# AgentMaker/PAPC

Measured on AMD Instinct MI355X. Metric: point-clouds/sec (fwd+bwd) PointNet++SSG B=32 N=4096, higher is better.
Workload: dtype f32

## Files before the change

include/papc_hip.h:

```cpp
#ifndef PAPC_HIP_H
#define PAPC_HIP_H

#include <stddef.h>
#include <stdint.h>

#ifdef __cplusplus
extern "C" {
#endif

#define PAPC_OK 0
#define PAPC_E_INVALID (-1)
#define PAPC_E_UNSUPPORTED (-2)
#define PAPC_E_LAUNCH (-3)

typedef void *papc_stream_t;

int papc_version(void);
#define PAPC_ABI_VERSION 8
int papc_abi_version(void);
int64_t papc_abi_sizeof(const char *struct_name);
const char *papc_last_error_string(void);


int papc_fps_f32(const float *xyz, int64_t sb, int64_t sn, int64_t sc, int B, int N, int npoint,
// ... 108 lines not shown
int papc_bn_eval_consts_f32(const float *running_mean, const float *running_var, const float *gamma, const float *beta,
                            float eps, int C, float *mean, float *invstd, float *scale, float *shift,
                            papc_stream_t stream);

int papc_group_max_bwd_f32(const float *gout, const int32_t *argmax, int64_t G, int K, int C, float *dx,
                           papc_stream_t stream);

typedef struct papc_bwd_dy {
    int dz_mode;
    const float *dz;
    const float *gout;
    const int32_t *argmax;
    int K;
    const float *y;
    const float *mean, *invstd, *scale, *shift, *c1, *c2;
    const float *wrow;
    const int32_t *seg_grp;
    const int32_t *rows_dev;
    const float *psel;
} papc_bwd_dy;

typedef struct papc_scatter_dst {
    float *grad_feats;
    const int32_t *idx;
    int N, S, K, D;
    int col0;
} papc_scatter_dst;
typedef struct papc_bwd_red {
    const float *y;
    const float *mean, *invstd, *scale, *shift;
    float *red_partial;
    int32_t store_masked;
} papc_bwd_red;
int papc_mlp_bwd_dx_f32(const papc_bwd_dy *dy, const float *wt, int64_t M, int Cin, int Cout, float *dx,
                        const papc_scatter_dst *scatter, const papc_bwd_red *next_red, papc_stream_t stream);

int papc_mlp_bwd_dw_f32(const papc_bwd_dy *dy, int a_mode, const float *x, int64_t ldx,
                        const papc_group_src *grp, const float *bn_scale, const float *bn_shift, int64_t M,
                        int Cin, int Cout, int rows_per_chunk, float *dw_partial, float *db_partial,
                        int64_t part_ld, papc_stream_t stream);

int papc_mlp_bwd_dw_chunk_hint(int64_t M, int Cin, int Cout, int a_mode, int dz_mode, int K);

int papc_reduce_partials_f32(const float *partial, int n_chunks, int64_t n, float *out, int accumulate,
                             papc_stream_t stream);
typedef struct papc_reduce_job {
    const float *partial;
    int32_t n_chunks;
    int32_t accumulate;
    int64_t ld, n1, n2;
    float *out1, *out2;
} papc_reduce_job;
int papc_reduce_partials_batch_f32(const papc_reduce_job *jobs, int count, papc_stream_t stream);
int papc_reduce_partials2_f32(const float *partial, int n_chunks, int64_t ld, int64_t n1, float *out1, int64_t n2,
                              float *out2, int accumulate, papc_stream_t stream);

#define PAPC_FOLD_MAX 24
typedef struct papc_fold_job {
    const float *partial;
    int32_t n_chunks;
    int32_t accumulate;
    int64_t ld;
    int32_t rows, cols;
    float *out; int64_t out_ld;
} papc_fold_job;
typedef struct papc_fold_list { papc_fold_job *jobs; int32_t capacity, count; } papc_fold_list;
int papc_fold_jobs_f32(const papc_fold_job *jobs, int count, papc_stream_t stream);

#define PAPC_SA_MAX_LAYERS 8
#define PAPC_SA_IN_GROUP 0
#define PAPC_SA_IN_ROWS 1
#define PAPC_SA_NO_LINGATHER 1u
#define PAPC_SA_NO_XYZ1 2u
#define PAPC_SA_NO_NOSTORE 4u
#define PAPC_SA_NO_GMAX 8u
#define PAPC_SA_NO_FUSED_RED 16u
#define PAPC_SA_NO_COMPACT 32u
#define PAPC_SA_NO_PLANES 64u
#define PAPC_SA_NO_PLANES_POINTWISE 128u
#define PAPC_SA_NO_XYZ_FUSE 256u
#define PAPC_SA_NO_PSEL 1024u
#define PAPC_SA_NO_GSIGN 2048u
#define PAPC_SA_NO_WSTATS 512u
typedef struct papc_sa_desc {
    int32_t B, N, S, K, D;
    int32_t n_layers;
    int32_t cin;
    int32_t cout[PAPC_SA_MAX_LAYERS];
    int32_t input;
    int32_t identity_rows;
    int32_t xyz_first, pool, eval_bn, cut_gather_grad;
    float eps, momentum;
    uint32_t disable;
    int32_t inference;
    int32_t want_input_grad;
} papc_sa_desc;
typedef struct papc_sa_layer {
    const float *w, *b, *gamma, *beta;
    float *running_mean, *running_var;
} papc_sa_layer;
typedef struct papc_compact_src {
    const int32_t *start, *rows, *cidx, *seg_grp;
    const float *wrow, *coef;
    int32_t G;
} papc_compact_src;
typedef struct papc_sa_io {
    const float *xyz; int64_t sb, sn, sc;
    const float *new_xyz;
    const float *feats;
    const int32_t *idx;
    const float *x_rows;
    const float *xc; const double *xc_gram;
    const papc_compact_src *compact;
    const float *consts3; int32_t consts3_ld;
    papc_sa_layer layer[PAPC_SA_MAX_LAYERS];
    float *out;
    void *saved, *scratch;
    const papc_point_lists *plists;
    const float *wfeat;
} papc_sa_io;
typedef struct papc_sa_plan {
    papc_sa_desc d;
    int32_t cin0;
    int32_t lin0, xyz1, gmax, nostore, compact, sparse_max, planes;
    int64_t saved_bytes, fwd_scratch_bytes, bwd_scratch_bytes;
    int64_t off_y[PAPC_SA_MAX_LAYERS], off_cst[PAPC_SA_MAX_LAYERS], off_argmax;
} papc_sa_plan;
typedef struct papc_sa_grads {
    const float *gout;
    float *dw[PAPC_SA_MAX_LAYERS], *db[PAPC_SA_MAX_LAYERS], *dgamma[PAPC_SA_MAX_LAYERS], *dbeta[PAPC_SA_MAX_LAYERS];
    int32_t acc_w[PAPC_SA_MAX_LAYERS], acc_gb[PAPC_SA_MAX_LAYERS];
    const float *wt[PAPC_SA_MAX_LAYERS];
    float *grad_feats, *grad_x;
    struct papc_fold_list *defer;
} papc_sa_grads;
int papc_sa_mlp_plan(const papc_sa_desc *desc, const papc_sa_io *io, papc_sa_plan *plan);
int papc_sa_mlp_fwd(const papc_sa_plan *plan, const papc_sa_io *io, papc_stream_t stream);
int papc_sa_mlp_bwd(const papc_sa_plan *plan, const papc_sa_io *io, const papc_sa_grads *grads, papc_stream_t stream);

typedef struct papc_pfn_desc {
    int32_t P, T, C;
    float vx, vy, x_offset, y_offset;
    float eps, momentum;
    int32_t training;
    int32_t zero_padded;
} papc_pfn_desc;
typedef struct papc_pfn_io {
    const float *features; const int32_t *num_voxels, *coors;
    const float *w, *gamma, *beta;
    float *running_mean, *running_var;
    float *out;
    void *saved, *scratch;
    uint32_t *tickets;
} papc_pfn_io;
int papc_pfn_workspace(const papc_pfn_desc *desc, int64_t *saved_bytes, int64_t *scratch_bytes);
int papc_pfn_fwd(const papc_pfn_desc *desc, const papc_pfn_io *io, papc_stream_t stream);
int papc_pfn_bwd(const papc_pfn_desc *desc, const papc_pfn_io *io, const float *gout, float *dw, float *dgamma, float *dbeta, int accumulate,
                 papc_stream_t stream);


int papc_pfn_decorate_f32(const float *features, const int32_t *num_voxels, const int32_t *coors, int P, int T,
                          float vx, float vy, float x_offset, float y_offset, int with_distance, float *out,
                          papc_stream_t stream);
int papc_pfn_decorate_nf_f32(const float *features, int F, const int32_t *num_voxels, const int32_t *coors, int P, int T,
                             float vx, float vy, float x_offset, float y_offset, int with_distance, float *out, papc_stream_t stream);
int papc_pfn_stats_f32(const float *features, const int32_t *num_voxels, const int32_t *coors, int P, int T,
// ... 22 lines not shown
                               float *running_mean, float *running_var, double *gram, papc_stream_t stream);
int papc_pfn_bwd_sparse_f32(const float *features, const int32_t *num_voxels, const int32_t *coors, int P,
                            int T, float vx, float vy, float x_offset, float y_offset, const float *w, int C,
                            const float *gout, const int32_t *argmax, const float *mean, const float *invstd,
                            const float *scale, const float *shift, float *partial, papc_stream_t stream);
int papc_pfn_bwd_finalize_f32(const float *sums, int64_t M, const float *w, int C, const double *gram, const float *mean,
                              const float *invstd, const float *scale, float *dgamma, float *dbeta, float *dw, int flags,
                              papc_stream_t stream);


size_t papc_points_to_voxel_workspace(int N);
int papc_points_to_voxel_f32(const float *points, int N, int ndim, const float *voxel_size, const float *coors_range,
                             int max_points, int max_voxels, int reverse_index, float *voxels, int32_t *coors,
                             int32_t *num_points, int32_t *voxel_num, void *workspace, size_t workspace_bytes,
                             papc_stream_t stream);

int papc_pillar_scatter_f32(const float *voxel_features, const int32_t *coords, int P, int C, int batch_size, int ny,
                            int nx, float *canvas, int32_t *owner, papc_stream_t stream);
int papc_pillar_scatter_bwd_f32(const float *grad_canvas, const int32_t *coords, const int32_t *owner, int P, int C,
                                int batch_size, int ny, int nx, float *grad_features, papc_stream_t stream);

int papc_head_fc_f32(const float *x, const float *w, const float *bias, const float *gamma, const float *beta, int B, int Cin, int Cout,
                     int has_bn, float eps, float momentum, float *running_mean, float *running_var, int64_t *num_batches_tracked,
                     float drop_p, const int64_t *rng_state, int layer_tag, int64_t *rng_bump, float *y, float *mean, float *invstd,
                     uint8_t *keep, float *out, papc_stream_t stream);
int papc_head_bwd_f32(const float *gnext, const float *wnext, int Cn, const float *out, const float *y, const float *mean,
                      const float *invstd, const float *gamma, float drop_p, int has_bn, const float *x, int B, int Cin, int Cout,
                      float *dy, float *dw, float *db, float *dgamma, float *dbeta, int accumulate, papc_stream_t stream);
int papc_softmax_xent_f32(const float *logits, const int64_t *labels, int B, int C, float *loss, float *dlogits, papc_stream_t stream);

typedef struct papc_head_fc_layer {
    const float *x, *w, *bias, *gamma, *beta;
    int32_t Cin, Cout, has_bn;
    float eps, momentum;
    float *running_mean, *running_var; int64_t *num_batches_tracked;
    float drop_p; int32_t layer_tag;
    float *y, *mean, *invstd; uint8_t *keep; float *out;
} papc_head_fc_layer;
typedef struct papc_head_bwd_job {
    const float *gnext, *wnext; int32_t Cn;
    const float *out, *y, *mean, *invstd, *gamma; float drop_p; int32_t has_bn;
    const float *x; int32_t Cin, Cout;
    float *dy, *dw, *db, *dgamma, *dbeta; int32_t accumulate;
    int32_t phase;
} papc_head_bwd_job;
int papc_head_chain_fwd_f32(const papc_head_fc_layer *layers, int n_layers, int B, const int64_t *rng_state, int64_t *rng_bump,
                            const int64_t *labels, float *loss, float *dlogits, uint32_t *sync, papc_stream_t stream);
int papc_head_chain_bwd_f32(const papc_head_bwd_job *jobs, int n_jobs, int B, uint32_t *sync, papc_stream_t stream);

int papc_cloud_transform_f32(const float *x, int64_t sb, int64_t sn, int64_t sc, const float *T, int64_t ldt, int B, int N, int C, float *y,
                             papc_stream_t stream);
size_t papc_cloud_transform_bwd_workspace(int B, int N, int C);
int papc_cloud_transform_bwd_f32(const float *x, int64_t sb, int64_t sn, int64_t sc, const float *T, int64_t ldt, const float *dy, int B, int N, int C,
                                 float *dx, int64_t dsb, int64_t dsn, int64_t dsc, int accumulate, float *dT, void *workspace,
                                 size_t workspace_bytes, papc_stream_t stream);

int papc_cloud_concat_conv_parts(int B, int N);
int papc_cloud_concat_conv_f32(const float *x, int64_t ldx, const float *g, const float *w, const float *bias, int B, int N, int Cp, int Cg, int Cout,
                               float *y, float *cvec, float *stats_partial, papc_stream_t stream);
size_t papc_cloud_concat_conv_bwd_workspace(int B, int N, int Cp, int Cg, int Cout);
int papc_cloud_concat_conv_bwd_f32(const float *dz, const float *y, const float *mean, const float *invstd, const float *scale, const float *shift,
                                   const float *c1, const float *c2, const float *x, int64_t ldx, const float *g, const float *w, int B, int N, int Cp,
                                   int Cg, int Cout, float *dx, int64_t ldd, int accumulate, float *dw, float *dbias, float *dg, float *s_out,
                                   void *workspace, size_t workspace_bytes, papc_stream_t stream);

size_t papc_nms_workspace(int N);
int papc_nms_f32(const float *dets, int N, float nms_overlap_thresh, int32_t *keep, int32_t *num_out, void *workspace,
                 size_t workspace_bytes, papc_stream_t stream);
int papc_rotate_nms_f32(const float *dets, int N, float nms_overlap_thresh, int32_t *keep, int32_t *num_out, void *workspace,
                        size_t workspace_bytes, papc_stream_t stream);
int papc_rotate_iou_f32(const float *boxes, const float *query_boxes, int N, int K, int criterion, float *iou, papc_stream_t stream);
int papc_rbbox_iou_f32(const float *box_corners, const float *qbox_corners, const float *standup_iou, float standup_thresh, int N, int K,
                       float *overlaps, papc_stream_t stream);
int papc_riou_f32(const float *rbboxes, const float *qrbboxes, float standup_thresh, int N, int K, float *overlaps, papc_stream_t stream);

int papc_lingather_parts(int64_t M);
int papc_mlp_compact_ok(int64_t M, int K, int n_layers, const int *couts);
int papc_compact_plan_f32(const int32_t *idx, int G, int K, int32_t *cnt8, int32_t *start, int32_t *rows, int32_t *cidx, int32_t *seg_grp,
                          float *wrow, float *coef, papc_stream_t stream);
int papc_compact_corr_parts(void);
int papc_bn_stats_corr_f32(const float *y, int C, const int32_t *start, const float *coef, int G, float *stats_rows, papc_stream_t stream);
int papc_bn_relu_max_seg_f32(const float *y, int C, const int32_t *start, const float *scale, const float *shift, int G, float *out,
                             int32_t *argmax, float *ysel, papc_stream_t stream);
int papc_lingather_fwd_f32(const float *P, const papc_group_src *grp, int B, const float *w, int ldw, int xcol0, const float *bias, int C,
                           float *y, float *stats_partial, papc_stream_t stream);
int papc_lingather_bwd_f32(const papc_bwd_dy *dy, const papc_group_src *grp, int B, int C, float *G, float *dwx_partial, papc_stream_t stream);
int papc_lingather_bwd_pp_ok(const papc_group_src *grp, int B, int C);
int papc_lingather_bwd_pp_f32(const papc_bwd_dy *dy, const papc_group_src *grp, int B, int C, const float *P, const float *w, int ldw, int xcol0,
                              const float *bias, float *G, float *dwx_partial, papc_stream_t stream);
int papc_lingather_list_parts(int64_t BN);
int papc_lingather_bwd_parts(const papc_group_src *grp, int B, int C);
int papc_lingather_bwd_lists_ok(const papc_group_src *grp, int C);
int papc_point_lists_f32(const papc_group_src *grp, int B, const int32_t *start, int32_t *prange, int32_t *prow, float *pmeta, float *pmom,
                         papc_stream_t stream);

int papc_mlp_bwd_dx_xyz_ok(int64_t M, int Cin, int Cout);
int papc_mlp_bwd_dx_xyz_f32(const papc_bwd_dy *dy, const float *wt, int64_t M, int Cin, int Cout, const float *xc, const float *wf,
                            float *partial, papc_stream_t stream);

int papc_bn_max_prep_f32(const float *gout, const float *ysel, const float *scale, const float *shift, const float *mean,
                         const float *invstd, const float *c1, const float *c2, const float *w, const float *bias, int64_t G, int Co,
                         int Ci, float *psel, float *wcat, float *hbias, float *e_out, float *q_out, papc_stream_t stream);
int papc_mlp_bwd_dx_max_f32(const float *psel, const int32_t *argmax, int K, const float *x, int64_t ldx, const float *bn_scale,
                            const float *bn_shift, const float *wcat, const float *hbias, int64_t M, int Cin, int Cout, float *dx,
                            const papc_bwd_red *next_red, papc_stream_t stream);

int papc_mlp_max_nostore_ok(int64_t M, int Cin, int Cout, int K);
int64_t papc_mlp_bwd_dw_max_ws_floats(int64_t M, int Cin, int Cout);
int papc_mlp_bwd_dw_max_f32(const float *psel, const int32_t *argmax, int K, const float *x, const float *bn_scale, const float *bn_shift,
                            const float *w, const float *e, const float *scale, const float *c1, int64_t M, int Cin, int Cout,
                            float *workspace, float *dw, int accumulate, papc_stream_t stream);

int papc_mlp_xyz_ok(int64_t M, int C1, int C2);
int papc_xyz_parts(int64_t M);
int papc_xyz_bwd_parts(int64_t M);
int papc_xyz_group_f32(const papc_group_src *grp, int B, float *xc, double *gram_partial, papc_stream_t stream);
int papc_xyz_gram_fold_f32(const double *gram_partial, int parts, double *gram, papc_stream_t stream);
int papc_xyz_l1_finalize_f32(const double *gram_partial, int parts, int64_t M, const float *w, int ldw, int xcol0, const float *bias,
                             const float *gamma, const float *beta, float eps, float momentum, int C, float *mean, float *invstd, float *scale,
                             float *shift, float *running_mean, float *running_var, float *wf, double *gram, papc_stream_t stream);
int papc_xyz_l1_bwd_f32(const float *dz, const float *xc, const float *wf, int64_t M, int C, float *partial, papc_stream_t stream);
int papc_xyz_l1_bwd_finalize_f32(const float *partial, int parts, int64_t M, int C, const double *gram, const float *w, int ldw, int xcol0,
                                 const float *bias, const float *mean, const float *invstd, const float *scale, float *dgamma, float *dbeta,
                                 float *dw, int accumulate, papc_stream_t stream);

size_t papc_pg_planes_bytes(int64_t R, int64_t K);

typedef struct papc_pg_wjob {
    const float *src;
    int64_t row_stride, col_stride;
    int R, K;
    void *planes;
} papc_pg_wjob;
int papc_pg_prep_weights_f32(const papc_pg_wjob *jobs, int count, papc_stream_t stream);

#define PAPC_PG_PLAIN 0
#define PAPC_PG_CONCAT 1
#define PAPC_PG_BNRELU 2
#define PAPC_PG_DY_DENSE 3
#define PAPC_PG_DY_MAX 4
typedef struct papc_pg_prep {
    int mode;
    int64_t M; int C;
    const float *x; int64_t ldx;
    const float *xyz; int64_t sb, sn, sc; const float *feats; int N, D, xyz_first;
    const float *dz;
    const float *gout, *ysel; const int32_t *argmax; int K;
    const float *stats; int parts;
    const float *gamma, *beta; float eps, momentum; float *running_mean, *running_var;
    float *mean, *invstd, *scale, *shift;
    const float *red; int red_parts;
    float *dgamma, *dbeta; int accumulate;
    void *planes, *planes_t;
} papc_pg_prep;
int papc_pg_prep_rows_f32(const papc_pg_prep *args, papc_stream_t stream);

#define PAPC_PG_STORE 0
#define PAPC_PG_FWD 1
#define PAPC_PG_FWD_GMAX 2
#define PAPC_PG_RED 3
typedef struct papc_pg_gemm {
    int epi;
    const void *a, *b;
    int R1, R2, K;
    float *c; int64_t ldc;
    int split; int64_t split_stride;
// ... 77 lines not shown
```

papc_amd/_lib.py:

```python
import ctypes
import os

_HERE = os.path.dirname(os.path.abspath(__file__))
LIB_PATH = os.environ.get("PAPC_LIB") or os.path.join(_HERE, "libpapc_hip.so")

ABI_VERSION = 8

c_p = ctypes.c_void_p
c_i = ctypes.c_int
c_l = ctypes.c_int64
c_f = ctypes.c_float


class PapcError(RuntimeError):
    pass


class GroupSrc(ctypes.Structure):
    _fields_ = [("xyz", c_p), ("sb", c_l), ("sn", c_l), ("sc", c_l), ("new_xyz", c_p), ("feats", c_p),
                ("idx", c_p), ("N", c_i), ("S", c_i), ("K", c_i), ("D", c_i), ("xyz_first", c_i),
                ("cidx", c_p), ("seg_grp", c_p), ("rows_dev", c_p), ("wstat", c_p), ("plists", c_p)]


class PointLists(ctypes.Structure):
    _fields_ = [("prange", c_p), ("prow", c_p), ("pmeta", c_p), ("compact", c_i), ("pmom", c_p)]


class BwdDy(ctypes.Structure):
    _fields_ = [("dz_mode", c_i), ("dz", c_p), ("gout", c_p), ("argmax", c_p), ("K", c_i), ("y", c_p),
                ("mean", c_p), ("invstd", c_p), ("scale", c_p), ("shift", c_p), ("c1", c_p), ("c2", c_p),
                ("wrow", c_p), ("seg_grp", c_p), ("rows_dev", c_p), ("psel", c_p)]


class GroupMax(ctypes.Structure):
    _fields_ = [("gmax", c_p), ("gmin", c_p), ("amax", c_p), ("amin", c_p), ("K", c_i), ("sign_src", c_p)]


class BwdRed(ctypes.Structure):
    _fields_ = [("y", c_p), ("mean", c_p), ("invstd", c_p), ("scale", c_p), ("shift", c_p), ("red_partial", c_p), ("store_masked", c_i)]


class CopyJob(ctypes.Structure):
    _fields_ = [("src", ctypes.c_void_p), ("dst", ctypes.c_void_p), ("B", ctypes.c_int32), ("R", ctypes.c_int32), ("C", ctypes.c_int32),
                ("sb", ctypes.c_int64), ("sr", ctypes.c_int64), ("sc", ctypes.c_int64), ("db", ctypes.c_int64), ("dr", ctypes.c_int64),
                ("dc", ctypes.c_int64)]


class ReduceJob(ctypes.Structure):
    _fields_ = [("partial", c_p), ("n_chunks", ctypes.c_int32), ("accumulate", ctypes.c_int32), ("ld", c_l), ("n1", c_l), ("n2", c_l),
                ("out1", c_p), ("out2", c_p)]


class ScatterDst(ctypes.Structure):
    _fields_ = [("grad_feats", c_p), ("idx", c_p), ("N", c_i), ("S", c_i), ("K", c_i), ("D", c_i), ("col0", c_i)]


SIGNATURES = {
    "papc_version": (c_i, []),
    "papc_abi_version": (c_i, []),
    "papc_abi_sizeof": (c_l, [ctypes.c_char_p]),
    "papc_last_error_string": (ctypes.c_char_p, []),
    "papc_fps_f32": (c_i, [c_p, c_l, c_l, c_l, c_i, c_i, c_i, c_p, c_f, c_p, c_p, c_p]),
    "papc_ball_query_f32": (c_i, [c_p, c_l, c_l, c_l, c_p, c_i, c_i, c_i, c_i, c_p, c_p, c_p, c_i, c_p]),
    "papc_square_distance_f32": (c_i, [c_p, c_p, c_i, c_i, c_i, c_p, c_p]),
    "papc_index_points_f32": (c_i, [c_p, c_p, c_i, c_i, c_i, c_i, c_i, c_p, c_p]),
    "papc_index_points_bwd_f32": (c_i, [c_p, c_p, c_i, c_i, c_i, c_i, c_i, c_p, c_p]),
    "papc_group_points_f32": (c_i, [c_p, c_l, c_l, c_l, c_p, c_p, c_p, c_i, c_i, c_i, c_i, c_i, c_i, c_p, c_p]),
    "papc_group_points_bwd_f32": (c_i, [c_p, c_p, c_i, c_i, c_i, c_i, c_i, c_i, c_p, c_p, c_p, c_p]),
    "papc_three_nn_f32": (c_i, [c_p, c_l, c_l, c_l, c_p, c_l, c_l, c_l, c_i, c_i, c_i, c_p, c_p, c_p, c_p]),
    "papc_three_interpolate_f32": (c_i, [c_p, c_p, c_p, c_i, c_i, c_i, c_i, c_p, c_p]),
    "papc_three_interpolate_bwd_f32": (c_i, [c_p, c_p, c_p, c_i, c_i, c_i, c_i, c_p, c_p]),
    "papc_three_interpolate_bwd_first3_f32": (c_i, [c_p, c_p, c_i, c_i, c_i, c_i, c_p, c_p]),
    "papc_mlp_gemm_parts": (c_i, [c_l]),
    "papc_mlp_gemm_gmax_ok": (c_i, [c_l, c_i, c_i]),
    "papc_mlp_gemm_f32": (c_i, [c_i, c_p, c_l, c_p, c_p, c_p, c_p, c_p, c_l, c_i, c_i, c_p, c_p, c_p, c_p]),
    "papc_mlp_gemm_rows_f32": (c_i, [c_i, c_p, c_l, c_p, c_p, c_p, c_p, c_p, c_l, c_i, c_i, c_p, c_p, c_p, c_p, c_p]),
    "papc_mlp_gemm_rows_w_f32": (c_i, [c_i, c_p, c_l, c_p, c_p, c_p, c_p, c_p, c_l, c_i, c_i, c_p, c_p, c_p, c_p, c_p, c_p]),
    "papc_sa_mlp_plan": (c_i, [c_p, c_p, c_p]),
    "papc_sa_mlp_fwd": (c_i, [c_p, c_p, c_p]),
    "papc_sa_mlp_bwd": (c_i, [c_p, c_p, c_p, c_p]),
    "papc_pfn_workspace": (c_i, [c_p, c_p, c_p]),
    "papc_pfn_fwd": (c_i, [c_p, c_p, c_p]),
    "papc_pfn_bwd": (c_i, [c_p, c_p, c_p, c_p, c_p, c_p, c_i, c_p]),
    "papc_compact_plan_f32": (c_i, [c_p, c_i, c_i, c_p, c_p, c_p, c_p, c_p, c_p, c_p, c_p]),
    "papc_compact_corr_parts": (c_i, []),
    "papc_mlp_compact_ok": (c_i, [c_l, c_i, c_i, c_p]),
    "papc_bn_stats_corr_f32": (c_i, [c_p, c_i, c_p, c_p, c_i, c_p, c_p]),
    "papc_bn_relu_max_seg_f32": (c_i, [c_p, c_i, c_p, c_p, c_p, c_i, c_p, c_p, c_p, c_p]),
    "papc_bn_select_max_f32": (c_i, [c_p, c_p, c_p, c_p, c_p, c_p, c_l, c_i, c_p, c_p, c_p]),
    "papc_bn_finalize_f32": (c_i, [c_p, c_i, c_l, c_i, c_p, c_p, c_f, c_f, c_p, c_p, c_p, c_p, c_p, c_p, c_p]),
    "papc_bn_relu_max_f32": (c_i, [c_p, c_p, c_p, c_l, c_i, c_i, c_p, c_p, c_p]),
    "papc_bn_relu_f32": (c_i, [c_p, c_p, c_p, c_l, c_i, c_p, c_p]),
    "papc_bn_bwd_reduce_max_f32": (c_i, [c_p, c_p, c_i, c_p, c_p, c_p, c_p, c_l, c_i, c_i, c_p, c_p, c_p]),
    "papc_bn_bwd_reduce_f32": (c_i, [c_i, c_p, c_p, c_p, c_i, c_p, c_p, c_p, c_p, c_p, c_l, c_i, c_i, c_p, c_p]),
    "papc_bn_bwd_finalize_f32": (c_i, [c_p, c_i, c_l, c_i, c_p, c_p, c_p, c_p, c_i, c_p]),
    "papc_bn_eval_consts_f32": (c_i, [c_p, c_p, c_p, c_p, c_f, c_i, c_p, c_p, c_p, c_p, c_p]),
    "papc_group_max_bwd_f32": (c_i, [c_p, c_p, c_l, c_i, c_i, c_p, c_p]),
    "papc_mlp_bwd_dx_f32": (c_i, [c_p, c_p, c_l, c_i, c_i, c_p, c_p, c_p, c_p]),
    "papc_mlp_bwd_dw_f32": (c_i, [c_p, c_i, c_p, c_l, c_p, c_p, c_p, c_l, c_i, c_i, c_i, c_p, c_p, c_l, c_p]),
    "papc_reduce_partials2_f32": (c_i, [c_p, c_i, c_l, c_l, c_p, c_l, c_p, c_i, c_p]),
    "papc_reduce_partials_batch_f32": (c_i, [c_p, c_i, c_p]),
    "papc_fold_jobs_f32": (c_i, [c_p, c_i, c_p]),
    "papc_mlp_bwd_dw_chunk_hint": (c_i, [c_l, c_i, c_i, c_i, c_i, c_i]),
    "papc_reduce_partials_f32": (c_i, [c_p, c_i, c_l, c_p, c_i, c_p]),
    "papc_pfn_decorate_f32": (c_i, [c_p, c_p, c_p, c_i, c_i, c_f, c_f, c_f, c_f, c_i, c_p, c_p]),
    "papc_pfn_decorate_nf_f32": (c_i, [c_p, c_i, c_p, c_p, c_i, c_i, c_f, c_f, c_f, c_f, c_i, c_p, c_p]),
    "papc_pfn_stats_f32": (c_i, [c_p, c_p, c_p, c_i, c_i, c_f, c_f, c_f, c_f, c_p, c_i, c_p, c_p, c_p]),
    "papc_pfn_apply_f32": (c_i, [c_p, c_p, c_p, c_i, c_i, c_f, c_f, c_f, c_f, c_p, c_i, c_p, c_p, c_p, c_p, c_p]),
    "papc_pfn_num_blocks": (c_i, [c_i]),
    "papc_pfn_bwd_reduce_f32": (c_i, [c_p, c_p, c_p, c_i, c_i, c_f, c_f, c_f, c_f, c_p, c_i, c_p, c_p, c_p, c_p, c_p, c_p, c_p, c_p]),
    "papc_pfn_bwd_dw_f32": (c_i, [c_p, c_p, c_p, c_i, c_i, c_f, c_f, c_f, c_f, c_p, c_i, c_p, c_p, c_p, c_p, c_p, c_p, c_p, c_p, c_p, c_p]),
    "papc_pfn_gram_blocks": (c_i, [c_i]),
    "papc_pfn_gram_f32": (c_i, [c_p, c_p, c_p, c_i, c_i, c_f, c_f, c_f, c_f, c_p, c_p]),
    "papc_pfn_gram_finalize_f32": (c_i, [c_p, c_i, c_l, c_p, c_i, c_p, c_p, c_f, c_f, c_p, c_p, c_p, c_p, c_p, c_p, c_p, c_p]),
    "papc_pfn_bwd_sparse_f32": (c_i, [c_p, c_p, c_p, c_i, c_i, c_f, c_f, c_f, c_f, c_p, c_i, c_p, c_p, c_p, c_p, c_p, c_p, c_p, c_p]),
    "papc_pfn_bwd_finalize_f32": (c_i, [c_p, c_l, c_p, c_i, c_p, c_p, c_p, c_p, c_p, c_p, c_p, c_i, c_p]),
    "papc_points_to_voxel_workspace": (ctypes.c_size_t, [c_i]),
    "papc_points_to_voxel_f32": (c_i, [c_p, c_i, c_i, c_p, c_p, c_i, c_i, c_i, c_p, c_p, c_p, c_p, c_p, ctypes.c_size_t, c_p]),
    "papc_pillar_scatter_f32": (c_i, [c_p, c_p, c_i, c_i, c_i, c_i, c_i, c_p, c_p, c_p]),
    "papc_pillar_scatter_bwd_f32": (c_i, [c_p, c_p, c_p, c_i, c_i, c_i, c_i, c_i, c_p, c_p]),
    "papc_head_fc_f32": (c_i, [c_p, c_p, c_p, c_p, c_p, c_i, c_i, c_i, c_i, c_f, c_f, c_p, c_p, c_p, c_f, c_p, c_i, c_p, c_p, c_p, c_p,
                               c_p, c_p, c_p]),
    "papc_head_bwd_f32": (c_i, [c_p, c_p, c_i, c_p, c_p, c_p, c_p, c_p, c_f, c_i, c_p, c_i, c_i, c_i, c_p, c_p, c_p, c_p, c_p, c_i, c_p]),
    "papc_softmax_xent_f32": (c_i, [c_p, c_p, c_i, c_i, c_p, c_p, c_p]),
    "papc_head_chain_fwd_f32": (c_i, [c_p, c_i, c_i, c_p, c_p, c_p, c_p, c_p, c_p, c_p]),
    "papc_head_chain_bwd_f32": (c_i, [c_p, c_i, c_i, c_p, c_p]),
    "papc_cloud_transform_f32": (c_i, [c_p, c_l, c_l, c_l, c_p, c_l, c_i, c_i, c_i, c_p, c_p]),
    "papc_cloud_transform_bwd_workspace": (ctypes.c_size_t, [c_i, c_i, c_i]),
    "papc_cloud_transform_bwd_f32": (c_i, [c_p, c_l, c_l, c_l, c_p, c_l, c_p, c_i, c_i, c_i, c_p, c_l, c_l, c_l, c_i, c_p, c_p, ctypes.c_size_t, c_p]),
    "papc_cloud_concat_conv_parts": (c_i, [c_i, c_i]),
    "papc_cloud_concat_conv_f32": (c_i, [c_p, c_l, c_p, c_p, c_p, c_i, c_i, c_i, c_i, c_i, c_p, c_p, c_p, c_p]),
    "papc_cloud_concat_conv_bwd_workspace": (ctypes.c_size_t, [c_i, c_i, c_i, c_i, c_i]),
    "papc_cloud_concat_conv_bwd_f32": (c_i, [c_p, c_p, c_p, c_p, c_p, c_p, c_p, c_p, c_p, c_l, c_p, c_p, c_i, c_i, c_i, c_i, c_i, c_p, c_l, c_i, c_p, c_p,
                                             c_p, c_p, c_p, ctypes.c_size_t, c_p]),
    "papc_nms_workspace": (ctypes.c_size_t, [c_i]),
    "papc_nms_f32": (c_i, [c_p, c_i, c_f, c_p, c_p, c_p, ctypes.c_size_t, c_p]),
    "papc_lingather_parts": (c_i, [c_l]),
    "papc_lingather_fwd_f32": (c_i, [c_p, c_p, c_i, c_p, c_i, c_i, c_p, c_i, c_p, c_p, c_p]),
    "papc_lingather_bwd_f32": (c_i, [c_p, c_p, c_i, c_i, c_p, c_p, c_p]),
    "papc_lingather_bwd_pp_f32": (c_i, [c_p, c_p, c_i, c_i, c_p, c_p, c_i, c_i, c_p, c_p, c_p, c_p]),
    "papc_lingather_list_parts": (c_i, [c_l]),
    "papc_lingather_bwd_parts": (c_i, [c_p, c_i, c_i]),
    "papc_lingather_bwd_lists_ok": (c_i, [c_p, c_i]),
    "papc_point_lists_f32": (c_i, [c_p, c_i, c_p, c_p, c_p, c_p, c_p, c_p]),
    "papc_lingather_bwd_pp_ok": (c_i, [c_p, c_i, c_i]),
    "papc_bn_max_prep_f32": (c_i, [c_p] * 10 + [c_l, c_i, c_i] + [c_p] * 6),
    "papc_mlp_max_nostore_ok": (c_i, [c_l, c_i, c_i, c_i]),
    "papc_mlp_bwd_dw_max_ws_floats": (c_l, [c_l, c_i, c_i]),
    "papc_mlp_bwd_dw_max_f32": (c_i, [c_p, c_p, c_i, c_p, c_p, c_p, c_p, c_p, c_p, c_p, c_l, c_i, c_i, c_p, c_p, c_i, c_p]),
    "papc_mlp_bwd_dx_xyz_ok": (c_i, [c_l, c_i, c_i]),
    "papc_mlp_bwd_dx_xyz_f32": (c_i, [c_p, c_p, c_l, c_i, c_i, c_p, c_p, c_p, c_p]),
    "papc_mlp_bwd_dx_max_f32": (c_i, [c_p, c_p, c_i, c_p, c_l, c_p, c_p, c_p, c_p, c_l, c_i, c_i, c_p, c_p, c_p]),
    "papc_mlp_xyz_ok": (c_i, [c_l, c_i, c_i]),
    "papc_xyz_parts": (c_i, [c_l]),
    "papc_xyz_bwd_parts": (c_i, [c_l]),
    "papc_xyz_group_f32": (c_i, [c_p, c_i, c_p, c_p, c_p]),
    "papc_xyz_gram_fold_f32": (c_i, [c_p, c_i, c_p, c_p]),
    "papc_xyz_l1_finalize_f32": (c_i, [c_p, c_i, c_l, c_p, c_i, c_i, c_p, c_p, c_p, c_f, c_f, c_i] + [c_p] * 9),
    "papc_xyz_l1_bwd_f32": (c_i, [c_p, c_p, c_p, c_l, c_i, c_p, c_p]),
    "papc_xyz_l1_bwd_finalize_f32": (c_i, [c_p, c_i, c_l, c_i, c_p, c_p, c_i, c_i] + [c_p] * 7 + [c_i, c_p]),
    "papc_pg_planes_bytes": (ctypes.c_size_t, [c_l, c_l]),
    "papc_pg_prep_weights_f32": (c_i, [c_p, c_i, c_p]),
    "papc_pg_prep_rows_f32": (c_i, [c_p, c_p]),
    "papc_pg_gemm_f32": (c_i, [c_p, c_p]),
    "papc_pg_gemm_group_f32": (c_i, [c_p, c_i, c_p]),
    "papc_pg_final_f32": (c_i, [c_p, c_i, c_l, c_i, c_p, c_p, c_f, c_f] + [c_p] * 10 + [c_l, c_p, c_p, c_p]),
    "papc_pg_final_groups_f32": (c_i, [c_p, c_i, c_l, c_i, c_p, c_p, c_f, c_f] + [c_p] * 10 + [c_l, c_i, c_p, c_p, c_p, c_p]),
    "papc_pg_fold_f32": (c_i, [c_p, c_i, c_p]),
    "papc_transpose_batch_f32": (c_i, [c_p, c_p, c_p, c_p, c_i, c_p]),
    "papc_transpose_batch_ld_f32": (c_i, [c_p, c_p, c_p, c_p, c_p, c_p, c_i, c_p]),
    "papc_rotate_nms_f32": (c_i, [c_p, c_i, c_f, c_p, c_p, c_p, ctypes.c_size_t, c_p]),
# ... 117 lines not shown
```

papc_amd/csrc/compact.hip:

```cpp
#include "common.h"

namespace papc {

__global__ __launch_bounds__(256) void compact_count_kernel(const int32_t *__restrict__ idx, int G, int K, int32_t *__restrict__ cnt8)
{
    const int g = blockIdx.x * 4 + (threadIdx.x >> 6), lane = threadIdx.x & 63;
    if (g >= G) return;
    const int32_t *row = idx + (int64_t)g * K;
    const int32_t first = row[0];
    int n = 0;
    for (int k = lane; k < K; k += 64) n += (k > 0 && row[k] != first) ? 1 : 0;
#pragma unroll
    for (int o = 32; o > 0; o >>= 1) n += __shfl_xor(n, o);
    if (lane == 0) cnt8[g] = (n + 1 + 7) & ~7;
}

__global__ __launch_bounds__(1024) void compact_scan_kernel(const int32_t *__restrict__ cnt8, int G, int32_t *__restrict__ start,
                                                            int32_t *__restrict__ rows)
{
    __shared__ int part[1024];
    const int tid = threadIdx.x;
    const int per = (G + 1023) / 1024;
    const int g0 = tid * per, g1 = min(G, g0 + per);
    int s = 0;
// ... 60 lines not shown
                }
#pragma unroll
                for (int u = 0; u < U; ++u) {
                    s1.x = fmaf(cf[u], v[u].x, s1.x); s1.y = fmaf(cf[u], v[u].y, s1.y); s1.z = fmaf(cf[u], v[u].z, s1.z); s1.w = fmaf(cf[u], v[u].w, s1.w);
                    s2.x = fmaf(cf[u] * v[u].x, v[u].x, s2.x); s2.y = fmaf(cf[u] * v[u].y, v[u].y, s2.y);
                    s2.z = fmaf(cf[u] * v[u].z, v[u].z, s2.z); s2.w = fmaf(cf[u] * v[u].w, v[u].w, s2.w);
                }
            }
        }
        red[0][threadIdx.x] = s1; red[1][threadIdx.x] = s2;
        __syncthreads();
        const int cqn = CQ < 256 ? CQ : 256;
        if ((int)threadIdx.x < cqn && c0 + (int)threadIdx.x < CQ) {
            float4 t1 = make_float4(0.f, 0.f, 0.f, 0.f), t2 = t1;
            for (int l = 0; l < RL; ++l) {
                const float4 a = red[0][l * cqn + threadIdx.x], b = red[1][l * cqn + threadIdx.x];
                t1.x += a.x; t1.y += a.y; t1.z += a.z; t1.w += a.w;
                t2.x += b.x; t2.y += b.y; t2.z += b.z; t2.w += b.w;
            }
            *reinterpret_cast<float4 *>(out + ((int64_t)r * 2 + 0) * C + 4 * (c0 + threadIdx.x)) = t1;
            *reinterpret_cast<float4 *>(out + ((int64_t)r * 2 + 1) * C + 4 * (c0 + threadIdx.x)) = t2;
        }
        __syncthreads();
    }
}

__global__ __launch_bounds__(256) void seg_max_kernel(const float *__restrict__ y, int C, const int32_t *__restrict__ start,
                                                      const float *__restrict__ scale, const float *__restrict__ shift, int G,
                                                      float *__restrict__ out, int32_t *__restrict__ argmax, float *__restrict__ ysel)
{
    const int CQ = C >> 2;
    const int64_t e = (int64_t)blockIdx.x * 256 + threadIdx.x;
    if (e >= (int64_t)G * CQ) return;
    const int g = (int)(e / CQ), c = (int)(e - (int64_t)g * CQ) * 4;
    const int r0 = start[g], r1 = start[g + 1];
    const float4 sc = *reinterpret_cast<const float4 *>(scale + c), sh = *reinterpret_cast<const float4 *>(shift + c);
    const float s4[4] = {sc.x, sc.y, sc.z, sc.w}, h4[4] = {sh.x, sh.y, sh.z, sh.w};
    int flip[4];
#pragma unroll
    for (int i = 0; i < 4; ++i) flip[i] = s4[i] >= 0.f ? 0 : (int)0x80000000u;
    float mx[4] = {-INFINITY, -INFINITY, -INFINITY, -INFINITY};
    int ix[4] = {r0, r0, r0, r0};
    const float *p = y + (int64_t)r0 * C + c;
    int r = r0;
    for (; r + 4 <= r1; r += 4) {
        float4 v[4];
#pragma unroll
        for (int u = 0; u < 4; ++u) v[u] = *reinterpret_cast<const float4 *>(p + (int64_t)u * C);
#pragma unroll
        for (int u = 0; u < 4; ++u) {
            const float a[4] = {v[u].x, v[u].y, v[u].z, v[u].w};
#pragma unroll
            for (int i = 0; i < 4; ++i) {
                const float k = __int_as_float(__float_as_int(a[i]) ^ flip[i]);
                if (k > mx[i]) { mx[i] = k; ix[i] = r + u; }
            }
        }
        p += (int64_t)4 * C;
    }
    for (; r < r1; ++r) {
        const float4 v = *reinterpret_cast<const float4 *>(p);
        const float a[4] = {v.x, v.y, v.z, v.w};
#pragma unroll
        for (int i = 0; i < 4; ++i) {
            const float k = __int_as_float(__float_as_int(a[i]) ^ flip[i]);
            if (k > mx[i]) { mx[i] = k; ix[i] = r; }
        }
        p += C;
    }
    float o[4], ys[4];
    int am[4];
#pragma unroll
    for (int i = 0; i < 4; ++i) {
        ys[i] = __int_as_float(__float_as_int(mx[i]) ^ flip[i]);
        am[i] = ix[i];
        o[i] = relu_np(fmaf(s4[i], ys[i], h4[i]));
    }
    const int64_t q = (int64_t)g * C + c;
    *reinterpret_cast<float4 *>(out + q) = make_float4(o[0], o[1], o[2], o[3]);
    *reinterpret_cast<int4 *>(argmax + q) = make_int4(am[0], am[1], am[2], am[3]);
    *reinterpret_cast<float4 *>(ysel + q) = make_float4(ys[0], ys[1], ys[2], ys[3]);
}

}

using namespace papc;

extern "C" {

int papc_compact_plan_f32(const int32_t *idx, int G, int K, int32_t *cnt8, int32_t *start, int32_t *rows, int32_t *cidx, int32_t *seg_grp,
                          float *wrow, float *coef, papc_stream_t stream)
{
    PAPC_REQUIRE(idx && cnt8 && start && rows && cidx && seg_grp && wrow && coef, PAPC_E_INVALID, "papc_compact_plan_f32: null pointer");
    PAPC_REQUIRE(G >= 1 && K >= 8 && K % 8 == 0, PAPC_E_UNSUPPORTED, "papc_compact_plan_f32: G=%d, nsample=%d must be a multiple of 8", G, K);
    PAPC_REQUIRE((int64_t)G * K < (1ll << 31), PAPC_E_UNSUPPORTED, "papc_compact_plan_f32: >= 2^31 rows");
    hipStream_t st = as_stream(stream);
    ProfScope prof(PAPC_K_GROUP, st);
    const unsigned nb = (unsigned)cdiv(G, 4);
    hipLaunchKernelGGL(compact_count_kernel, dim3(nb), dim3(256), 0, st, idx, G, K, cnt8);
    hipLaunchKernelGGL(compact_scan_kernel, dim3(1), dim3(1024), 0, st, cnt8, G, start, rows);
    hipLaunchKernelGGL(compact_fill_kernel, dim3(nb), dim3(256), 0, st, idx, G, K, start, rows, cidx, seg_grp, wrow, coef);
    return check_launch("papc_compact_plan_f32");
}

int papc_compact_corr_parts(void) { return 64; }

int papc_bn_stats_corr_f32(const float *y, int C, const int32_t *start, const float *coef, int G, float *stats_rows, papc_stream_t stream)
{
    PAPC_REQUIRE(y && start && coef && stats_rows, PAPC_E_INVALID, "papc_bn_stats_corr_f32: null pointer");
    PAPC_REQUIRE(G >= 1 && C >= 4 && C % 4 == 0 && aligned16(y) && aligned16(stats_rows), PAPC_E_INVALID, "papc_bn_stats_corr_f32: C %% 4 == 0 and 16-byte aligned rows");
    hipStream_t st = as_stream(stream);
    ProfScope prof(PAPC_K_MISC, st);
    hipLaunchKernelGGL(bn_stats_corr_kernel, dim3((unsigned)papc_compact_corr_parts()), dim3(256), 0, st, y, C, start, coef, G, stats_rows);
    return check_launch("papc_bn_stats_corr_f32");
}

int papc_bn_relu_max_seg_f32(const float *y, int C, const int32_t *start, const float *scale, const float *shift, int G, float *out,
                             int32_t *argmax, float *ysel, papc_stream_t stream)
{
    PAPC_REQUIRE(y && start && scale && shift && out && argmax && ysel, PAPC_E_INVALID, "papc_bn_relu_max_seg_f32: null pointer");
    PAPC_REQUIRE(G >= 1 && C >= 4 && C % 4 == 0, PAPC_E_UNSUPPORTED, "papc_bn_relu_max_seg_f32: C=%d must be a multiple of 4", C);
    PAPC_REQUIRE(aligned16(y) && aligned16(scale) && aligned16(shift) && aligned16(out) && aligned16(argmax) && aligned16(ysel), PAPC_E_INVALID,
                 "papc_bn_relu_max_seg_f32: 16-byte alignment");
    hipStream_t st = as_stream(stream);
    ProfScope prof(PAPC_K_BN_RELU_MAX, st);
    hipLaunchKernelGGL(seg_max_kernel, dim3((unsigned)cdiv((int64_t)G * (C / 4), 256)), dim3(256), 0, st, y, C, start, scale, shift, G, out, argmax, ysel);
    return check_launch("papc_bn_relu_max_seg_f32");
}

}
```

papc_amd/csrc/mlp_gemm.h:

```cpp
#pragma once
#include "mlp_loaders.h"

namespace papc {

typedef float floatx16 __attribute__((ext_vector_type(16)));

enum { EPI_STORE = 0, EPI_SCATTER = 1, EPI_STORE_RED = 2, EPI_STORE_GMAX = 3, EPI_GMAX = 4, EPI_XYZ_RED = 5 };

struct RedSrc {
    const float *y; const float *mean, *invstd, *scale, *shift;
    int masked;
};

struct ScatterDst {
    float *gf; const int32_t *idx; int N, S, K, D;
    FastDiv divSK, divK;
};

struct GmaxDst {
    float *gmax, *gmin; int32_t *amax, *amin; int K;
    const float *sgn;
};

struct GemmArgs {
    ASrc a;
    const float *w; int64_t ldw;
    int wmap;
    int nmap;
    const float *bias;
    int64_t M; int Kin; int Nout;
    float *y; int64_t ldy;
    float *stats;
    int parts;
    ScatterDst sc;
    RedSrc rd;
    GmaxDst gm;
    const int32_t *rows_dev;
    const float *wstat;
    unsigned long long *dbg;
    int tl;
};

constexpr int GEMM_MAX_PARTS = 768;

int stream_gemm_try(const GemmArgs &p, int amode, int epi, bool vec, hipStream_t st);

}
```

papc_amd/csrc/mlp_gemm.hip:

```cpp
#include "mlp_gemm.h"
#include <mutex>
#include <unordered_map>

namespace papc {

constexpr int LDT = 36;
constexpr int BK = 32;

template <bool VEC, bool WMAP, bool NMAP>
__device__ __forceinline__ float4 fetch_w4(const GemmArgs &p, int n, int k)
{
    const int nn = n < p.Nout ? n : 0;
    const int nrow = NMAP ? gk(p.a.g, nn) : nn;
    const float *wr = p.w + (int64_t)nrow * p.ldw;
    float4 v;
    if (WMAP) {
        v.x = wr[k < p.Kin ? gk(p.a.g, k) : 0];
        v.y = wr[k + 1 < p.Kin ? gk(p.a.g, k + 1) : 0];
        v.z = wr[k + 2 < p.Kin ? gk(p.a.g, k + 2) : 0];
        v.w = wr[k + 3 < p.Kin ? gk(p.a.g, k + 3) : 0];
    } else if (VEC) {
        v = ld4(wr + (k < p.Kin ? k : 0));
    } else {
        v.x = wr[k < p.Kin ? k : 0];
// ... 860 lines not shown
    return PAPC_OK;
}

}

using namespace papc;

extern "C" {

int papc_mlp_gemm_parts(int64_t M) { return gemm_parts(M); }

int papc_mlp_gemm_gmax_ok(int64_t M, int Cout, int K)
{
    if (!(K == 32 || K == 64 || K == 128) || M % 128 != 0 || Cout <= 32 || Cout % 32 != 0) return 0;
    if (K == 128 && !(Cout == 64 || Cout % 128 == 0)) return 0;
    const int64_t gx = gemm_parts(M);
    if (Cout > 64 && gx * cdiv(Cout, 128) < 192 && gx * cdiv(Cout, 64) < 1024 && !(gx * cdiv(Cout, 64) >= 192)) return 0;
    return 1;
}

int papc_mlp_gemm_f32(int a_mode, const float *x, int64_t ldx, const papc_group_src *grp,
                      const float *bn_scale, const float *bn_shift, const float *w, const float *bias,
                      int64_t M, int Cin, int Cout, float *y, float *stats_partial, const papc_group_max *gmax,
                      papc_stream_t stream)
{
    return papc_mlp_gemm_rows_f32(a_mode, x, ldx, grp, bn_scale, bn_shift, w, bias, M, Cin, Cout, y, stats_partial, gmax, nullptr, stream);
}

int papc_mlp_gemm_rows_w_f32(int a_mode, const float *x, int64_t ldx, const papc_group_src *grp,
                           const float *bn_scale, const float *bn_shift, const float *w, const float *bias,
                           int64_t M, int Cin, int Cout, float *y, float *stats_partial, const papc_group_max *gmax,
                           const int32_t *rows_dev, const float *wrow, papc_stream_t stream)
{
    PAPC_REQUIRE(w && (y || gmax), PAPC_E_INVALID, "papc_mlp_gemm_f32: null w/y");
    PAPC_REQUIRE(!rows_dev || (!gmax && (a_mode == A_PLAIN || a_mode == A_BNRELU)), PAPC_E_UNSUPPORTED,
                 "papc_mlp_gemm_rows_f32: a device-side row count goes with plain / BN+ReLU rows and no fused group max");
    PAPC_REQUIRE(M >= 1 && Cin >= 1 && Cout >= 1, PAPC_E_INVALID, "papc_mlp_gemm_f32: M=%lld Cin=%d Cout=%d", (long long)M, Cin, Cout);
    PAPC_REQUIRE(M < (1ll << 31), PAPC_E_UNSUPPORTED, "papc_mlp_gemm_f32: M=%lld >= 2^31 rows", (long long)M);
    GemmArgs p;
    memset(&p, 0, sizeof(p));
    int rc = fill_asrc(p.a, a_mode, x, ldx, grp, bn_scale, bn_shift, Cin, "papc_mlp_gemm_f32");
    if (rc) return rc;
    p.w = w; p.ldw = Cin; p.bias = bias; p.M = M; p.Kin = Cin; p.Nout = Cout; p.y = y; p.ldy = Cout; p.stats = stats_partial;
    p.rows_dev = rows_dev;
    p.wstat = rows_dev ? wrow : nullptr;
    p.wmap = (a_mode == A_GROUP) ? 1 : 0;
    const bool vec = p.a.vec && (p.wmap || (aligned16(w) && Cin % 4 == 0));
    hipStream_t st = as_stream(stream);
    ProfScope prof(PAPC_K_MLP_GEMM, st);
    PAPC_REQUIRE(!(gmax && a_mode == A_XYZ), PAPC_E_UNSUPPORTED, "papc_mlp_gemm_f32: PAPC_A_XYZ has no fused group-max flavour");
    if (gmax) {
        PAPC_REQUIRE(gmax->gmax && gmax->gmin && gmax->amax && gmax->amin, PAPC_E_INVALID, "papc_mlp_gemm_f32: null pointer in gmax");
        PAPC_REQUIRE(papc_mlp_gemm_gmax_ok(M, Cout, gmax->K), PAPC_E_UNSUPPORTED,
                     "papc_mlp_gemm_f32: fused group max needs K in {32,64,128}, M %% 128 == 0, Cout > 32 (got K=%d M=%lld Cout=%d)",
                     gmax->K, (long long)M, Cout);
        p.gm.gmax = gmax->gmax; p.gm.gmin = gmax->gmin; p.gm.amax = gmax->amax; p.gm.amin = gmax->amin; p.gm.K = gmax->K; p.gm.sgn = gmax->sign_src;
        if (!y) {
            GemmArgs q = p;
            q.parts = gemm_parts(p.M);
            const int rc2 = a_mode == A_BNRELU ? stream_gemm_try(q, A_BNRELU, EPI_GMAX, vec, st) : 0;
            if (rc2 == 0) { set_error("papc_mlp_gemm_f32: y = NULL (no stored output under the max) is not built for a_mode=%d M=%lld Cin=%d Cout=%d K=%d", a_mode, (long long)M, Cin, Cout, gmax->K); return PAPC_E_UNSUPPORTED; }
            return rc2 < 0 ? rc2 : PAPC_OK;
        }
        switch (a_mode) {
        case A_PLAIN: return launch_gemm<A_PLAIN, EPI_STORE_GMAX>(p, vec, st);
        case A_BNRELU: return launch_gemm<A_BNRELU, EPI_STORE_GMAX>(p, vec, st);
        default: return launch_gemm<A_GROUP, EPI_STORE_GMAX>(p, vec, st);
        }
    }
    if (a_mode == A_XYZ) {
        GemmArgs q = p;
        q.parts = gemm_parts(p.M);
        const int rc2 = stream_gemm_try(q, A_XYZ, EPI_STORE, vec, st);
        if (rc2 == 0) { set_error("papc_mlp_gemm_f32: PAPC_A_XYZ is not built for M=%lld Cin=%d Cout=%d", (long long)M, Cin, Cout); return PAPC_E_UNSUPPORTED; }
        return rc2 < 0 ? rc2 : PAPC_OK;
    }
    switch (a_mode) {
    case A_PLAIN: return launch_gemm<A_PLAIN, EPI_STORE>(p, vec, st);
    case A_BNRELU: return launch_gemm<A_BNRELU, EPI_STORE>(p, vec, st);
    default: return launch_gemm<A_GROUP, EPI_STORE>(p, vec, st);
    }
}

int papc_mlp_gemm_rows_f32(int a_mode, const float *x, int64_t ldx, const papc_group_src *grp,
                           const float *bn_scale, const float *bn_shift, const float *w, const float *bias,
                           int64_t M, int Cin, int Cout, float *y, float *stats_partial, const papc_group_max *gmax,
                           const int32_t *rows_dev, papc_stream_t stream)
{
    return papc_mlp_gemm_rows_w_f32(a_mode, x, ldx, grp, bn_scale, bn_shift, w, bias, M, Cin, Cout, y, stats_partial, gmax, rows_dev, nullptr, stream);
}

int papc_mlp_xyz_ok(int64_t M, int C1, int C2)
{
    if (!knob(KNOB_STREAM) || knob(KNOB_GEMM_F32) || !knob(KNOB_DW_ROWS) || knob(KNOB_DW_F32)) return 0;
    if (M % 64 != 0 || M / 32 < knob(KNOB_STREAM_MINTILES)) return 0;
    if (C1 != 64 || !(C2 == 64 || C2 == 128)) return 0;
    if (M * (int64_t)C2 * 4 >= (1ll << 32)) return 0;
    if ((C1 / 64) * (C2 / 64) > knob(KNOB_DW_ROWS_BLOCKS)) return 0;
    return 1;
}

int papc_mlp_max_nostore_ok(int64_t M, int Cin, int Cout, int K)
{
    if (!knob(KNOB_STREAM) || knob(KNOB_GEMM_F32) || !knob(KNOB_STREAM_ASM) || !knob(KNOB_STREAM_MAXCAT) || !knob(KNOB_DW_ROWS) || knob(KNOB_DW_F32)) return 0;
    if (!knob(KNOB_MAX_NOSTORE)) return 0;
    if (M % 128 != 0 || M / 32 < knob(KNOB_STREAM_MINTILES) || M * (int64_t)Cout * 4 >= (1ll << 32)) return 0;
    if (!(K == 32 || K == 64 || K == 128) || !papc_mlp_gemm_gmax_ok(M, Cout, K)) return 0;
    if (!(Cin == 64 && Cout == 128)) return 0;
    return 1;
}

int papc_mlp_compact_ok(int64_t M, int K, int n_layers, const int *couts)
{
    if (!knob(KNOB_STREAM) || knob(KNOB_GEMM_F32) || !knob(KNOB_STREAM_ASM) || !knob(KNOB_DW_ROWSX) || knob(KNOB_DW_F32)) return 0;
    if (!couts || n_layers < 2 || M % 128 != 0 || M / 32 < knob(KNOB_STREAM_MINTILES) || K < 8 || K % 8 != 0) return 0;
    if (M * 256 * 4 >= (1ll << 32)) return 0;
    if (couts[0] != 128) return 0;
    for (int l = 1; l < n_layers; ++l)
        if (couts[l] != (l == n_layers - 1 ? 256 : 128)) return 0;
    return 1;
}

int papc_mlp_bwd_dx_f32(const papc_bwd_dy *dy, const float *wt, int64_t M, int Cin, int Cout, float *dx,
                        const papc_scatter_dst *scatter, const papc_bwd_red *next_red, papc_stream_t stream)
{
    PAPC_REQUIRE(wt, PAPC_E_INVALID, "papc_mlp_bwd_dx_f32: null wt");
    PAPC_REQUIRE(dx || scatter, PAPC_E_INVALID, "papc_mlp_bwd_dx_f32: need dx or scatter");
    PAPC_REQUIRE(M >= 1 && Cin >= 1 && Cout >= 1, PAPC_E_INVALID, "papc_mlp_bwd_dx_f32: bad sizes");
    PAPC_REQUIRE(M < (1ll << 31), PAPC_E_UNSUPPORTED, "papc_mlp_bwd_dx_f32: M=%lld >= 2^31 rows", (long long)M);
    bool vec = false;
    int rc = check_dy(dy, M, Cout, &vec, "papc_mlp_bwd_dx_f32");
    if (rc) return rc;
    GemmArgs p;
    memset(&p, 0, sizeof(p));
    fill_dy(p.a.d, dy);
    p.a.d.C = Cout;
    p.w = wt; p.ldw = Cout; p.M = M; p.Kin = Cout; p.Nout = Cin; p.y = dx; p.ldy = Cin;
    vec = vec && aligned16(wt);
    if (scatter) {
        PAPC_REQUIRE(scatter->grad_feats && scatter->D >= 1 && scatter->D + 3 == Cin, PAPC_E_INVALID,
                     "papc_mlp_bwd_dx_f32: scatter needs grad_feats and D+3 == Cin");
        PAPC_REQUIRE(scatter->N >= 1 && scatter->S >= 1 && scatter->K >= 1, PAPC_E_INVALID, "papc_mlp_bwd_dx_f32: scatter bad N/S/K");
        p.sc.gf = scatter->grad_feats; p.sc.idx = scatter->idx; p.sc.N = scatter->N; p.sc.S = scatter->S;
        p.sc.K = scatter->K; p.sc.D = scatter->D;
        p.sc.divSK = make_fastdiv((uint32_t)scatter->S * (uint32_t)scatter->K);
        p.sc.divK = make_fastdiv((uint32_t)scatter->K);
        p.nmap = scatter->col0 ? 1 : 0;
        p.a.g.D = scatter->D; p.a.g.xyz_first = scatter->col0 ? 1 : 0;
        p.Nout = scatter->D;
    }
    if (next_red) {
        PAPC_REQUIRE(!scatter && dx, PAPC_E_INVALID, "papc_mlp_bwd_dx_f32: next_red needs a dense dx");
        PAPC_REQUIRE(next_red->y && next_red->mean && next_red->invstd && next_red->scale && next_red->shift && next_red->red_partial,
                     PAPC_E_INVALID, "papc_mlp_bwd_dx_f32: null pointer in next_red");
        p.rd.y = next_red->y; p.rd.mean = next_red->mean; p.rd.invstd = next_red->invstd; p.rd.scale = next_red->scale;
        p.rd.shift = next_red->shift; p.stats = next_red->red_partial; p.rd.masked = next_red->store_masked ? 1 : 0;
    }
    const int tl_on = knob(KNOB_GEMM_TL);
    p.tl = tl_on && !scatter && dx && aligned16(dx) && Cin % 4 == 0 && (!next_red || (aligned16(next_red->y) && Cin <= 64 && !next_red->store_masked));
    hipStream_t st = as_stream(stream);
    ProfScope prof(PAPC_K_BWD_DX, st);
    if (next_red) {
        return dy->dz_mode == PAPC_DZ_DENSE ? launch_gemm<A_DY_DENSE, EPI_STORE_RED>(p, vec, st) : launch_gemm<A_DY_MAX, EPI_STORE_RED>(p, vec, st);
    }
    if (scatter) {
        return dy->dz_mode == PAPC_DZ_DENSE ? launch_gemm<A_DY_DENSE, EPI_SCATTER>(p, vec, st) : launch_gemm<A_DY_MAX, EPI_SCATTER>(p, vec, st);
// ... 70 lines not shown
```

papc_amd/csrc/mlp_stream.hip:

```cpp
#include "mlp_gemm.h"
#include <type_traits>
#include <utility>

namespace papc {

typedef float f32x4 __attribute__((ext_vector_type(4)));

template <int I, int N, class F>
__device__ __forceinline__ void sfor(F &&f)
{
    if constexpr (I < N) {
        f(std::integral_constant<int, I>{});
        sfor<I + 1, N>(f);
    }
}

template <bool ASM, int OFF, bool FIRST>
__device__ __forceinline__ void gload4(f32x4 &d, unsigned voff, const char *sbase)
{
    if constexpr (ASM) {
        if constexpr (FIRST) asm volatile("s_nop 4\n\tglobal_load_dwordx4 %0, %1, %2 offset:%3" : "+v"(d) : "v"(voff), "s"(sbase), "n"(OFF));
        else asm volatile("global_load_dwordx4 %0, %1, %2 offset:%3" : "+v"(d) : "v"(voff), "s"(sbase), "n"(OFF));
    } else {
        d = *reinterpret_cast<const f32x4 *>(sbase + voff + OFF);
    }
}
template <bool ASM, int N>
__device__ __forceinline__ void wait_vm()
{
    if constexpr (ASM) asm volatile("s_waitcnt vmcnt(%0)" ::"n"(N));
}
template <bool ASM>
__device__ __forceinline__ void touch(f32x4 &d)
{
    if constexpr (ASM) asm volatile("" : "+v"(d));
}

struct StreamGeo {
    int n_units;
    int ushift;
    int kgshift;
    const int *rows_dev;
    const float *wrow;
    const int *seg_grp;
    const float *wstat;
};

#ifndef PAPC_STREAM_PK
#define PAPC_STREAM_PK 1
#endif
typedef float f32x2 __attribute__((ext_vector_type(2)));
__device__ __forceinline__ f32x2 pk_fma(f32x2 a, f32x2 b, f32x2 c) { return __builtin_elementwise_fma(a, b, c); }
__device__ __forceinline__ void split3_pair(f32x2 x, unsigned &p0, unsigned &p1, unsigned &p2)
{
    p0 = pack_bf16x2(x.x, x.y);
    x = x - f32x2{bf16_lo(p0), bf16_hi(p0)};
    p1 = pack_bf16x2(x.x, x.y);
    x = x - f32x2{bf16_lo(p1), bf16_hi(p1)};
    p2 = pack_bf16x2(x.x, x.y);
}

template <int AMODE, int EPI, int KB16, int CK, int WN, bool ASM, bool CP = false, int KV = KB16 * 16, bool NR = false, int CBW = WN * 32, bool PS = false, int NWT = 8,
          bool GS = false>
__global__ __launch_bounds__(NWT * 64, NWT / 4) void stream_kernel(GemmArgs p, StreamGeo geo)
{
    static_assert(!GS || EPI == EPI_STORE_GMAX || EPI == EPI_GMAX, "GS: group-max epilogues only");
    static_assert(NWT == 8 || NWT == 12, "two or three waves per SIMD");
    static_assert(!PS || (CP && AMODE == A_DY_MAX), "PS: the compacted max-layer dX only (the one flavour where the result is bit-identical)");
    static_assert(!CP || ((AMODE == A_DY_DENSE || AMODE == A_DY_MAX) && EPI == EPI_STORE_RED && ASM && PAPC_STREAM_PK), "CP: dX flavours of the asm ring only");
    constexpr int NW = NWT;
    constexpr bool KR = (KV != KB16 * 16);
    constexpr int K = KR ? KV + 4 : KB16 * 16;
    constexpr int NT = WN * 32;
    constexpr int KBF = KR ? KB16 - 1 : KB16;
    static_assert(!KR || (KV == KB16 * 16 - 12 && !CP && PAPC_STREAM_PK && (AMODE == A_BNRELU || AMODE == A_DY_DENSE || AMODE == A_PLAIN)), "ragged k: four channels in the last block");
    static_assert(!NR || (EPI == EPI_STORE || EPI == EPI_STORE_RED), "ragged n: storing epilogues without the group max");
    constexpr int NCH = KBF / CK;
    static_assert(KBF % CK == 0 && NCH >= 2 && NCH % 2 == 0, "an even number of chunks per tile");
    constexpr bool DY = (AMODE == A_DY_DENSE || AMODE == A_DY_MAX);
    constexpr bool GM = (EPI == EPI_STORE_GMAX || EPI == EPI_GMAX);
    constexpr bool XYZ = (AMODE == A_XYZ);
    constexpr bool MC = (AMODE == A_MAXCAT);
    constexpr int KS = MC ? KB16 * 2 / 3 : 0;
    static_assert(!MC || (KB16 % 3 == 0 && CK == 1), "MAXCAT: Cout = 2 Cin, one k block per chunk");
    constexpr int NLD = (AMODE == A_DY_MAX) ? 6 : ((AMODE == A_DY_DENSE || MC) ? 4 : 2);
    constexpr int NLDP = KR ? NLD / 2 : 0;
    constexpr int CLB = CK * NLD;
    constexpr int CL = CLB + NLDP;
    static_assert(CL <= 60, "vmcnt is a 6-bit field");
    constexpr int ROWB = 6 * K + (KR ? 32 : 16);
    static_assert((ROWB / 16) % 2 == 1 && ROWB % 16 == 0, "conflict-free fragment reads");
    constexpr int NCST = (AMODE == A_BNRELU || MC) ? 2 : (DY ? 5 : (XYZ ? 4 : 0));
    constexpr bool CB = (CBW != NT);
    constexpr int TB = CBW / 32;
    static_assert(!CB || (NR && TB == WN - 1 && CBW % 32 != 0), "a narrow column block ends inside its last tile");
    constexpr int NROW = CB ? CBW + 1 : NT;
    constexpr int W_BYTES = NROW * ROWB;
    constexpr int CST_BYTES = NCST * K * 4 + (KR ? 32 : 0);
    constexpr bool XR = (EPI == EPI_XYZ_RED);
    constexpr int NSUM = XR ? 4 : 2;
    constexpr int RED_BYTES = NSUM * NW * NT * 4;
    constexpr int SMEM = (W_BYTES + CST_BYTES) > RED_BYTES ? (W_BYTES + CST_BYTES) : RED_BYTES;
    __shared__ __attribute__((aligned(16))) char smem[SMEM];
    char *cstb = smem + W_BYTES;

    const int tid = threadIdx.x, lane = tid & 63;
    const int wave = __builtin_amdgcn_readfirstlane(tid >> 6);
    const int hi = lane >> 5, l31 = lane & 31;
    const int n0 = blockIdx.y * CBW;
    const int ldx = (int)(DY ? p.a.d.C : p.a.ldx);
    auto nld_of = [](int ci) constexpr -> int { return MC ? ((ci % NCH) < KS ? 4 : 2) : (CK * NLD + ((ci % NCH) == NCH - 1 ? NLDP : 0)); };

    {
        const float *wb = p.w + (int64_t)n0 * p.ldw;
        constexpr int NP = NROW * (K / 4);
        constexpr int NI = (NP + NW * 64 - 1) / (NW * 64);
        constexpr bool PG = (NP % (NW * 64) != 0);
        static_assert(KR || CB || !PG || NW != 8, "whole float4 pieces per thread");
        float4 wv[NI];
#pragma unroll
        for (int q = 0; q < NI; ++q) {
            const int i = tid + q * NW * 64;
            const int n = i / (K / 4), k4 = (i - n * (K / 4)) * 4;
            bool ok = true;
            if constexpr (KR) ok = ok && k4 < KV;
            if constexpr (PG) ok = ok && i < NP;
            if constexpr (NR) ok = ok && n0 + n < p.Nout;
            if constexpr (CB) ok = ok && n < CBW;
            wv[q] = ok ? ld4(wb + (int64_t)n * p.ldw + k4) : make_float4(0.f, 0.f, 0.f, 0.f);
        }
#pragma unroll
        for (int q = 0; q < NI; ++q) {
            const int i = tid + q * NW * 64;
            const int n = i / (K / 4), k4 = (i - n * (K / 4)) * 4;
            uint2 q0, q1, q2;
            split3(wv[q], q0, q1, q2);
            char *d = smem + n * ROWB + k4 * 2;
            if (!PG || i < NP) {
                *reinterpret_cast<uint2 *>(d) = q0;
                *reinterpret_cast<uint2 *>(d + 2 * K) = q1;
                *reinterpret_cast<uint2 *>(d + 4 * K) = q2;
            }
        }
        if constexpr (KR) {
            for (int n = tid; n < NROW; n += NW * 64) {
                *reinterpret_cast<uint4 *>(smem + n * ROWB + 6 * K) = make_uint4(0u, 0u, 0u, 0u);
                *reinterpret_cast<uint4 *>(smem + n * ROWB + 6 * K + 16) = make_uint4(0u, 0u, 0u, 0u);
            }
        }
// ... 245 lines not shown
            if constexpr (AMODE == A_PLAIN) {
#pragma unroll
                for (int i = 0; i < 4; ++i) { v[i] = r[0][i]; v[4 + i] = r[1][i]; }
            } else if constexpr (AMODE == A_BNRELU) {
                const f32x4 s0 = *reinterpret_cast<const f32x4 *>(cl + kb * 64), s1 = *reinterpret_cast<const f32x4 *>(cl + kb * 64 + 16);
                const f32x4 h0 = *reinterpret_cast<const f32x4 *>(cl + K * 4 + kb * 64), h1 = *reinterpret_cast<const f32x4 *>(cl + K * 4 + kb * 64 + 16);
#pragma unroll
                for (int i = 0; i < 4; ++i) {
                    v[i] = fmaxf(fmaf(s0[i], r[0][i], h0[i]), 0.f);
                    v[4 + i] = fmaxf(fmaf(s1[i], r[1][i], h1[i]), 0.f);
                }
            } else {
                f32x4 c[5][2];
#pragma unroll
                for (int q = 0; q < 5; ++q) {
                    c[q][0] = *reinterpret_cast<const f32x4 *>(cl + q * K * 4 + kb * 64);
                    c[q][1] = *reinterpret_cast<const f32x4 *>(cl + q * K * 4 + kb * 64 + 16);
                }
#pragma unroll
                for (int h = 0; h < 2; ++h)
#pragma unroll
                    for (int i = 0; i < 4; ++i) {
                        const float y = r[h][i];
                        float dz = r[2 + h][i];
                        if constexpr (AMODE == A_DY_MAX) dz = (__float_as_int(r[4 + h][i]) == kin) ? dz : 0.f;
                        const float z = fmaf(c[0][h][i], y, c[1][h][i]);
                        const float pp = z > 0.f ? dz : 0.f;
                        v[4 * h + i] = fmaf(-c[4][h][i], y - c[2][h][i], fmaf(c[0][h][i], pp, -c[3][h][i]));
                    }
            }
            uint2 a0, a1, a2, b0, b1, b2;
            split3(make_float4(v[0], v[1], v[2], v[3]), a0, a1, a2);
            split3(make_float4(v[4], v[5], v[6], v[7]), b0, b1, b2);
            af[0] = __builtin_bit_cast(bf16x8, make_uint4(a0.x, a0.y, b0.x, b0.y));
            af[1] = __builtin_bit_cast(bf16x8, make_uint4(a1.x, a1.y, b1.x, b1.y));
            af[2] = __builtin_bit_cast(bf16x8, make_uint4(a2.x, a2.y, b2.x, b2.y));
#endif
            bf16x8 bq[WN][3];
#pragma unroll
            for (int wn = 0; wn < WN; ++wn)
#pragma unroll
                for (int pl = 0; pl < 3; ++pl)
                    bq[wn][pl] = *reinterpret_cast<const bf16x8 *>(((CB && wn == TB) ? wlb : wl + wn * 32 * ROWB) + pl * 2 * K + kb * 32);
            constexpr int PA[6] = {2, 1, 0, 1, 0, 0}, PB[6] = {0, 1, 2, 0, 1, 0};
#pragma unroll
            for (int t = 0; t < 6; ++t)
#pragma unroll
                for (int wn = 0; wn < WN; ++wn)
                    acc[wn] = __builtin_amdgcn_mfma_f32_32x32x16_bf16(af[PA[t]], bq[wn][PB[t]], acc[wn], 0, 0, 0);
        }
    };
    auto compute = [&](auto bi_, auto ci_) {
        constexpr int bi = decltype(bi_)::value, ci = decltype(ci_)::value;
        sfor<0, CK>([&](auto blk_) {
            constexpr int blk = decltype(blk_)::value;
            compute_block(std::integral_constant<int, ci * CK + blk>{}, &buf[bi][blk * NLD]);
        });
        if constexpr (KR && ci == NCH - 1) {
            const f32x4 z4 = f32x4{0.f, 0.f, 0.f, 0.f};
            f32x4 rr[4];
            rr[0] = pbuf[0]; rr[1] = z4;
            rr[2] = (AMODE == A_DY_DENSE) ? pbuf[NLDP - 1] : z4; rr[3] = z4;
            compute_block(std::integral_constant<int, KBF>{}, rr);
        }
    };

    float s1[WN], s2[WN], biasv[WN];
    float rsc[WN], rsh[WN], rmu[WN], ris[WN];
    float gmx[WN], gmn[WN];
    int gix[WN], gin[WN];
    float s3[WN], s4[WN];
    float4 kq[WN];
#pragma unroll
    for (int wn = 0; wn < WN; ++wn) {
        const int colr = n0 + wn * 32 + l31;
        const int col = NR ? min(colr, p.Nout - 1) : colr;
        s1[wn] = 0.f; s2[wn] = 0.f; s3[wn] = 0.f; s4[wn] = 0.f;
        kq[wn] = XR ? ld4(p.rd.scale + 4 * col) : make_float4(0.f, 0.f, 0.f, 0.f);
        biasv[wn] = (!CP && !(KR && DY) && p.bias && colr == col && (!CB || wn * 32 + l31 < CBW)) ? p.bias[col] : 0.f;
        rsc[wn] = rsh[wn] = rmu[wn] = ris[wn] = 0.f;
        if (EPI == EPI_STORE_RED) { rsc[wn] = p.rd.scale[col]; rsh[wn] = p.rd.shift[col]; rmu[wn] = p.rd.mean[col]; ris[wn] = p.rd.invstd[col]; }
        gmx[wn] = -INFINITY; gmn[wn] = INFINITY; gix[wn] = 0; gin[wn] = 0;
        if constexpr (GS) gin[wn] = (p.gm.sgn[col] < 0.f) ? (int)0x80000000u : 0;
    }

    auto epilogue = [&](int row0, int sub) {
        const int64_t ldy = p.ldy;
        if constexpr (XR) {
            const float4 *xq = reinterpret_cast<const float4 *>(p.rd.y) + row0 + 4 * hi;
#pragma unroll
            for (int g = 0; g < 4; ++g) {
                float4 xv[4];
#pragma unroll
                for (int i = 0; i < 4; ++i) xv[i] = xq[8 * g + i];
#pragma unroll
                for (int wn = 0; wn < WN; ++wn) {
#pragma unroll
                    for (int i = 0; i < 4; ++i) {
                        const int r = 4 * g + i;
                        const float z = fmaf(kq[wn].z, xv[i].z, fmaf(kq[wn].y, xv[i].y, fmaf(kq[wn].x, xv[i].x, kq[wn].w)));
                        const float pp = z > 0.f ? acc[wn][r] : 0.f;
                        s1[wn] = fmaf(pp, xv[i].x, s1[wn]); s2[wn] = fmaf(pp, xv[i].y, s2[wn]); s3[wn] = fmaf(pp, xv[i].z, s3[wn]);
                        s4[wn] += pp;
                        acc[wn][r] = 0.f;
                    }
                }
                __builtin_amdgcn_sched_barrier(0);
            }
            return;
        }
#pragma unroll
        for (int wn = 0; wn < WN; ++wn) {
            const int col = n0 + wn * 32 + l31;
            const bool cok = (!NR || col < p.Nout) && (!CB || wn * 32 + l31 < CBW);
            float *yp = p.y + (int64_t)(row0 + 4 * hi) * ldy + col;
            if (EPI == EPI_STORE_RED) {
                if (cok) {
                const float *qp = p.rd.y + (int64_t)(row0 + 4 * hi) * ldy + col;
                float yv[16];
#pragma unroll
                for (int r = 0; r < 16; ++r) yv[r] = qp[(int64_t)((r & 3) + 8 * (r >> 2)) * ldy];
#pragma unroll
                for (int r = 0; r < 16; ++r) {
                    const float v = acc[wn][r] + biasv[wn];
                    const float pp = fmaf(rsc[wn], yv[r], rsh[wn]) > 0.f ? v : 0.f;
                    if constexpr (CP) yp[(int64_t)((r & 3) + 8 * (r >> 2)) * ldy] = pp;
                    else yp[(int64_t)((r & 3) + 8 * (r >> 2)) * ldy] = v;
                    s1[wn] += pp;
                    s2[wn] = fmaf(pp, (yv[r] - rmu[wn]) * ris[wn], s2[wn]);
                    if constexpr (CP) { if ((r & 3) == 3) __builtin_amdgcn_sched_barrier(0); }
                }
                }
            } else {
#pragma unroll
                for (int r = 0; r < 16; ++r) {
                    const int ro = (r & 3) + 8 * (r >> 2);
                    const float v = acc[wn][r] + biasv[wn];
                    if (EPI != EPI_GMAX && cok) yp[(int64_t)ro * ldy] = v;
                    s1[wn] += v;
                    s2[wn] = fmaf(v, v, s2[wn]);
                    if (GM) {
                        const int off = sub * 32 + ro + 4 * hi;
                        if constexpr (GS) {
                            const float key = __int_as_float(__float_as_int(v) ^ gin[wn]);
                            if (key > gmx[wn]) { gmx[wn] = key; gix[wn] = off; }
                        } else {
                            if (v > gmx[wn]) { gmx[wn] = v; gix[wn] = off; }
                            if (v < gmn[wn]) { gmn[wn] = v; gin[wn] = off; }
                        }
                    }
                }
            }
#pragma unroll
            for (int r = 0; r < 16; ++r) acc[wn][r] = 0.f;
            if (GM && sub == U - 1) {
                if constexpr (GS) {
                    float vmx = gmx[wn];
                    int imx = gix[wn];
                    const float omx = __shfl_xor(vmx, 32);
                    const int oix = __shfl_xor(imx, 32);
                    if (omx > vmx || (omx == vmx && oix < imx)) { vmx = omx; imx = oix; }
                    if (hi == 0) {
                        const int64_t g = (int64_t)(row0 >> 5) >> geo.ushift;
                        const float sel = __int_as_float(__float_as_int(vmx) ^ gin[wn]);
                        p.gm.gmax[g * p.Nout + col] = sel; p.gm.amax[g * p.Nout + col] = imx;
                        p.gm.gmin[g * p.Nout + col] = sel; p.gm.amin[g * p.Nout + col] = imx;
                    }
                    gmx[wn] = -INFINITY; gix[wn] = 0;
                } else {
                float vmx = gmx[wn], vmn = gmn[wn];
                int imx = gix[wn], imn = gin[wn];
                const float omx = __shfl_xor(vmx, 32), omn = __shfl_xor(vmn, 32);
                const int oix = __shfl_xor(imx, 32), oin = __shfl_xor(imn, 32);
                if (omx > vmx || (omx == vmx && oix < imx)) { vmx = omx; imx = oix; }
                if (omn < vmn || (omn == vmn && oin < imn)) { vmn = omn; imn = oin; }
                if (hi == 0) {
                    const int64_t g = (int64_t)(row0 >> 5) >> geo.ushift;
                    p.gm.gmax[g * p.Nout + col] = vmx; p.gm.amax[g * p.Nout + col] = imx;
                    p.gm.gmin[g * p.Nout + col] = vmn; p.gm.amin[g * p.Nout + col] = imn;
                }
                gmx[wn] = -INFINITY; gmn[wn] = INFINITY; gix[wn] = 0; gin[wn] = 0;
                }
            }
        }
    };

    if constexpr (XYZ) {
        if (my_tiles > 0) {
            const float4 *xc = reinterpret_cast<const float4 *>(p.a.x);
            int row0 = tile_row0(0);
            float4 xn = xc[row0 + l31];
            for (int j = 0; j < my_tiles; ++j) {
                const float4 xv = xn;
                const int row0n = tile_row0(j + 1);
                xn = xc[row0n + l31];
                asm volatile("" ::: "memory");
                sfor<0, KB16>([&](auto kb_) { compute_xyz(kb_, xv); });
                epilogue(row0, j & (U - 1));
                row0 = row0n;
            }
        }
    }
    if (!XYZ && my_tiles > 0) {
        int row0 = tile_row0(0);
        SB sa = bases(row0);
        unsigned vgnxt = voff_grp0;
        auto vg_of = [&](int g) -> unsigned { return (unsigned)((g * ldx + 8 * hi) * 4); };
        if constexpr (CP) {
            const int r1 = tile_row0(1);
            wcur = -geo.wrow[row0 + l31];
            if constexpr (AMODE == A_DY_MAX) {
                sa.vg = vg_of(geo.seg_grp[(row0 + l31) >> 3]);
                vgnxt = vg_of(geo.seg_grp[(r1 + l31) >> 3]);
            }
        }
        issue(std::integral_constant<int, 0>{}, std::integral_constant<int, 0>{}, sa);
        issue(std::integral_constant<int, 1>{}, std::integral_constant<int, 1>{}, sa);
        wait_vm<ASM, nld_of(1)>();
        touch_buf(std::integral_constant<int, 0>{});
        for (int j = 0; j < my_tiles; ++j) {
            const int row0n = tile_row0(j + 1);
            SB sn = bases(row0n);
            if constexpr (CP) sn.vg = vgnxt;
            if (AMODE == A_DY_MAX || MC) kin = CP ? row0 + l31 : (row0 & ((1 << geo.kgshift) - 1)) + l31;
#ifdef PAPC_STREAM_NO_LATE1
            constexpr bool LATE1 = false;
#else
            constexpr bool LATE1 = (EPI == EPI_STORE_RED || EPI == EPI_XYZ_RED);
#endif
            sfor<0, NCH>([&](auto c_) {
                constexpr int c = decltype(c_)::value;
                constexpr int bi = c & 1;
                if constexpr (c > 0) {
// ... 31 lines not shown

    if constexpr (EPI == EPI_STORE && (AMODE == A_BNRELU || AMODE == A_PLAIN) && !NR && !KR) {
        if (geo.wstat && p.stats && my_tiles > 0) {
            asm volatile("s_waitcnt vmcnt(0)" ::: "memory");
            for (int j = 0; j < my_tiles; ++j) {
                const int row0 = tile_row0(j);
                float cfq[2], vq[2][WN];
#pragma unroll
                for (int q = 0; q < 2; ++q) {
                    const int64_t row = row0 + 8 * (2 * q + hi);
                    cfq[q] = geo.wstat[row] - 1.f;
#pragma unroll
                    for (int wn = 0; wn < WN; ++wn) vq[q][wn] = p.y[row * p.ldy + n0 + wn * 32 + l31];
                }
#pragma unroll
                for (int q = 0; q < 2; ++q)
#pragma unroll
                    for (int wn = 0; wn < WN; ++wn) {
                        s1[wn] = fmaf(cfq[q], vq[q][wn], s1[wn]);
                        s2[wn] = fmaf(cfq[q] * vq[q][wn], vq[q][wn], s2[wn]);
                    }
            }
        }
    }

    if (p.stats) {
        __syncthreads();
        float *red = reinterpret_cast<float *>(smem);
#pragma unroll
        for (int wn = 0; wn < WN; ++wn) {
            s1[wn] += __shfl_xor(s1[wn], 32);
            s2[wn] += __shfl_xor(s2[wn], 32);
            if (XR) { s3[wn] += __shfl_xor(s3[wn], 32); s4[wn] += __shfl_xor(s4[wn], 32); }
            if (hi == 0) {
                red[(0 * NW + wave) * NT + wn * 32 + l31] = s1[wn];
                red[(1 * NW + wave) * NT + wn * 32 + l31] = s2[wn];
                if (XR) {
                    red[(2 * NW + wave) * NT + wn * 32 + l31] = s3[wn];
                    red[(3 * NW + wave) * NT + wn * 32 + l31] = s4[wn];
                }
            }
        }
        __syncthreads();
        for (int i = tid; i < NSUM * NT; i += NW * 64) {
            const int which = i / NT, c = i - which * NT;
            float t = 0.f;
#pragma unroll
            for (int w = 0; w < NW; ++w) t += red[(which * NW + w) * NT + c];
            const int64_t col_off = XR ? (int64_t)(n0 + c) * 4 + which : (int64_t)which * p.Nout + n0 + c;
            const int64_t row_ld = (int64_t)NSUM * p.Nout;
            if ((NR && n0 + c >= p.Nout) || (CB && c >= CBW)) continue;
            p.stats[(int64_t)blockIdx.x * row_ld + col_off] = t;
            for (int r = blockIdx.x + gridDim.x; r < p.parts; r += gridDim.x) p.stats[(int64_t)r * row_ld + col_off] = 0.f;
        }
    }
}

static int stream_ncu()
{
    static int ncu = 0;
    if (!ncu) {
        int dev = 0;
        hipDeviceProp_t prop;
        if (hipGetDevice(&dev) == hipSuccess && hipGetDeviceProperties(&prop, dev) == hipSuccess && prop.multiProcessorCount > 0) ncu = prop.multiProcessorCount;
        else ncu = 256;
    }
    return ncu;
}

template <int AMODE, int EPI, int KB16, int WN, bool CP = false, int KV = KB16 * 16, bool NR = false, int CBW = WN * 32, bool PS = false>
static int stream_go(const GemmArgs &p, const StreamGeo &geo, hipStream_t st)
{
    constexpr bool KR = (KV != KB16 * 16);
    constexpr int KBF = KR ? KB16 - 1 : KB16;
    constexpr int CK2 = (KBF == 6) ? 1 : 2;
    constexpr int CK = (KBF < 4 || AMODE == A_DY_MAX || AMODE == A_MAXCAT || (AMODE == A_DY_DENSE && (WN == 4 || KR)) || (AMODE == A_PLAIN && KB16 == 8 && WN == 4)) ? 1 : CK2;
    const int ncb = (p.Nout + CBW - 1) / CBW;
    int gx = std::max(8, (stream_ncu() / ncb) & ~7);
    if (!CP && (AMODE == A_MAXCAT || AMODE == A_XYZ)) gx *= 2;
    gx = std::min(gx, std::max(1, (geo.n_units + 7) / 8));
    if (gx > p.parts) gx = p.parts;
    dim3 grid((unsigned)gx, (unsigned)ncb);
    if constexpr (!CP && EPI == EPI_STORE_RED) { if (p.rd.masked) return 0; }
    if constexpr (CP) {
        if (!knob(KNOB_STREAM_ASM)) return 0;
        if constexpr (PS) {
            GemmArgs q = p;
            q.a.d.gout = p.a.d.psel;
            hipLaunchKernelGGL((stream_kernel<AMODE, EPI, KB16, CK, WN, true, true, KB16 * 16, false, WN * 32, true>), grid, dim3(512), 0, st, q, geo);
        } else {
            hipLaunchKernelGGL((stream_kernel<AMODE, EPI, KB16, CK, WN, true, true>), grid, dim3(512), 0, st, p, geo);
        }
        const int rc = check_launch("mlp stream gemm (compacted)");
        return rc ? rc : 1;
    }
    if constexpr (AMODE == A_XYZ) hipLaunchKernelGGL((stream_kernel<AMODE, EPI, KB16, CK, WN, false>), grid, dim3(512), 0, st, p, geo);
    else if (knob(KNOB_STREAM_ASM)) {
        if constexpr ((EPI == EPI_XYZ_RED || (EPI == EPI_STORE_RED && AMODE == A_DY_MAX && KB16 == 16)) && WN == 2 && !NR && KV == KB16 * 16) {
            if (knob(KNOB_STREAM_NW12)) hipLaunchKernelGGL((stream_kernel<AMODE, EPI, KB16, CK, WN, true, false, KV, NR, CBW, false, 12>), grid, dim3(768), 0, st, p, geo);
            else hipLaunchKernelGGL((stream_kernel<AMODE, EPI, KB16, CK, WN, true, false, KV, NR, CBW>), grid, dim3(512), 0, st, p, geo);
        } else if constexpr ((EPI == EPI_GMAX || EPI == EPI_STORE_GMAX) && !NR && KV == KB16 * 16) {
            if (p.gm.sgn) hipLaunchKernelGGL((stream_kernel<AMODE, EPI, KB16, CK, WN, true, false, KV, NR, CBW, false, 8, true>), grid, dim3(512), 0, st, p, geo);
            else hipLaunchKernelGGL((stream_kernel<AMODE, EPI, KB16, CK, WN, true, false, KV, NR, CBW>), grid, dim3(512), 0, st, p, geo);
        } else {
            hipLaunchKernelGGL((stream_kernel<AMODE, EPI, KB16, CK, WN, true, false, KV, NR, CBW>), grid, dim3(512), 0, st, p, geo);
        }
    }
    else if constexpr (AMODE == A_MAXCAT || EPI == EPI_GMAX || EPI == EPI_XYZ_RED || KR || NR) return 0;
    else hipLaunchKernelGGL((stream_kernel<AMODE, EPI, KB16, CK, WN, false>), grid, dim3(512), 0, st, p, geo);
    const int rc = check_launch("mlp stream gemm");
    return rc ? rc : 1;
}

template <int AMODE, int EPI>
static int stream_pick(const GemmArgs &p, const StreamGeo &geo, hipStream_t st)
{
    const int kb = p.Kin / 16;
    if (geo.wrow) {
        if constexpr (AMODE == A_DY_DENSE && EPI == EPI_STORE_RED) { if (kb == 8 && p.Nout == 128) return stream_go<AMODE, EPI, 8, 4, true>(p, geo, st); }
        if constexpr (AMODE == A_DY_MAX && EPI == EPI_STORE_RED) {
            if (kb == 16 && p.Nout == 128) {
                if (p.a.d.psel) return stream_go<AMODE, EPI, 16, 2, true, 256, false, 64, true>(p, geo, st);
                return stream_go<AMODE, EPI, 16, 2, true>(p, geo, st);
            }
        }
        return 0;
    }
    if (geo.wstat && (p.Kin == 196 || p.Nout == 196)) return 0;
    if (p.Kin == 196 || p.Nout == 196) {
        if constexpr (AMODE == A_BNRELU && EPI == EPI_STORE) { if (p.Kin == 128 && p.Nout == 196) return stream_go<AMODE, EPI, 8, 4, false, 128, true>(p, geo, st); }
        if constexpr (AMODE == A_BNRELU && (EPI == EPI_STORE_GMAX || EPI == EPI_STORE)) { if (p.Kin == 196 && p.Nout % 128 == 0) return stream_go<AMODE, EPI, 13, 4, false, 196>(p, geo, st); }
        if constexpr (AMODE == A_DY_MAX && EPI == EPI_STORE_RED) { if (p.Kin == 256 && p.Nout == 196) return stream_go<AMODE, EPI, 16, 4, false, 256, true, 98>(p, geo, st); }
        if constexpr (AMODE == A_DY_DENSE && EPI == EPI_STORE_RED) { if (p.Kin == 196 && p.Nout % 128 == 0) return stream_go<AMODE, EPI, 13, 4, false, 196>(p, geo, st); }
        return 0;
    }
    const int nt = p.Kin > 128 ? 64 : 128;
    int wn = std::min(p.Nout, nt) / 32;
    if (p.Nout % (32 * wn) != 0) {
        if (p.Nout == 96 && nt >= 96) wn = 3;
        else return 0;
    }
#define STREAM_CASE(KB, WNN) if (kb == KB && wn == WNN) return stream_go<AMODE, EPI, KB, WNN>(p, geo, st)
    if constexpr (EPI == EPI_GMAX) {
        STREAM_CASE(4, 4); STREAM_CASE(8, 4);
    } else if constexpr (AMODE == A_MAXCAT) {
        STREAM_CASE(12, 2); STREAM_CASE(24, 2);
    } else if constexpr (AMODE == A_XYZ) {
        STREAM_CASE(4, 2); STREAM_CASE(4, 4);
    } else if constexpr (AMODE == A_DY_DENSE && (EPI == EPI_STORE || EPI == EPI_XYZ_RED)) {
        STREAM_CASE(4, 2); STREAM_CASE(8, 2);
    } else {
        STREAM_CASE(2, 2); STREAM_CASE(2, 4);
        STREAM_CASE(4, 2); STREAM_CASE(4, 4);
        STREAM_CASE(8, 2); STREAM_CASE(8, 4);
        STREAM_CASE(4, 3); STREAM_CASE(8, 3);
        STREAM_CASE(6, 2); STREAM_CASE(6, 4);
        if constexpr (AMODE == A_DY_DENSE || AMODE == A_DY_MAX || AMODE == A_BNRELU) { STREAM_CASE(16, 2); }
    }
#undef STREAM_CASE
    return 0;
}

static int ilog2_exact(int v)
{
    int s = 0;
    while ((1 << s) < v) ++s;
// ... 46 lines not shown
```

papc_amd/csrc/sa_mlp.hip:

```cpp
#include "common.h"

#define SA_CALL(expr)                 \
    do {                              \
        const int rc__ = (expr);      \
        if (rc__ != PAPC_OK) return rc__; \
    } while (0)

namespace papc {
int pfn_gram_stats(const float *features, const int32_t *num_voxels, const int32_t *coors, int P, int T, float vx, float vy, float x_offset, float y_offset, int zero_padded,
                   double *gram_partial, const float *w, int C, const float *gamma, const float *beta, float eps, float momentum, float *mean, float *invstd,
                   float *scale, float *shift, float *running_mean, float *running_var, double *gram, unsigned *ticket, hipStream_t st);
int pfn_gram_impl(const float *features, const int32_t *num_voxels, const int32_t *coors, int P, int T, float vx, float vy, float x_offset, float y_offset,
                  double *gram_partial, int zero_padded, papc_stream_t stream);
int pfn_apply_impl(const float *features, const int32_t *num_voxels, const int32_t *coors, int P, int T, float vx, float vy, float x_offset, float y_offset,
                   const float *w, int C, const float *scale, const float *shift, float *out, int32_t *argmax, int zero_padded, papc_stream_t stream);
int pfn_bwd_sparse_impl(const float *features, const int32_t *num_voxels, const int32_t *coors, int P, int T, float vx, float vy, float x_offset, float y_offset,
                        const float *w, int C, const float *gout, const int32_t *argmax, const float *mean, const float *invstd, const float *scale,
                        const float *shift, float *partial, int zero_padded, papc_stream_t stream);
int pfn_bwd_fold_finalize(const float *partial, int n_chunks, float *sums, int64_t M, const float *w, int C, const double *gram, const float *mean,
                          const float *invstd, const float *scale, float *dgamma, float *dbeta, float *dw, int flags, unsigned *ticket, hipStream_t st);

constexpr int A_PLAIN_ = PAPC_A_PLAIN, A_BNRELU_ = PAPC_A_BNRELU, A_GROUP_ = PAPC_A_GROUP, A_XYZ_ = PAPC_A_XYZ;

struct Carver {
    char *base;
    size_t off;
    template <class T>
    T *take(size_t n)
    {
        off = (off + 255) & ~(size_t)255;
        T *p = base ? reinterpret_cast<T *>(base + off) : nullptr;
        off += n * sizeof(T);
        return p;
    }
};

struct SavedPtrs {
    float *y[PAPC_SA_MAX_LAYERS];
    float *cst[PAPC_SA_MAX_LAYERS];
    int32_t *argmax;
    float *gbuf_f;
    float *xc; double *gram; float *wf;
    float *P;
};
struct FwdPtrs {
    float *stats;
    int32_t *gbuf_i;
    float *P, *wfeat;
    double *gpart;
};
struct BwdPtrs {
    float *c12[PAPC_SA_MAX_LAYERS];
    float *wt[PAPC_SA_MAX_LAYERS];
    float *part[PAPC_SA_MAX_LAYERS];
    float *red, *fused_red[2];
    float *dz[2];
    float *psel, *wcat, *hb, *eq, *dwmax_ws;
    float *bpart;
    float *dwx_part, *Gs, *part_g, *wft;
    float *tmp_gb;
};

static inline int64_t rows_of(const papc_sa_desc &d) { return (int64_t)d.B * d.S * d.K; }

static bool defer_fold(const papc_sa_grads &gr, const float *partial, int n_chunks, int64_t ld, int rows, int cols, float *out, int64_t out_ld, int accumulate)
{
    papc_fold_list *fl = gr.defer;
    if (!fl || !fl->jobs || fl->count >= fl->capacity) return false;
    papc_fold_job &j = fl->jobs[fl->count++];
    j.partial = partial; j.n_chunks = n_chunks; j.accumulate = accumulate; j.ld = ld; j.rows = rows; j.cols = cols; j.out = out; j.out_ld = out_ld;
    return true;
}
static bool defer_room(const papc_sa_grads &gr, int n) { return gr.defer && gr.defer->jobs && gr.defer->count + n <= gr.defer->capacity; }
static inline int cin_of(const papc_sa_plan &p, int l) { return l == 0 ? p.cin0 : p.d.cout[l - 1]; }

static int dw_rows_per_chunk(int64_t M, int cout, int cin, int min_rows = 256)
{
    const bool wide = cin > 128 && cin <= 160;
    const int tiles = ((cout + 127) / 128) * (wide ? 1 : (cin + 127) / 128);
    const int want = std::max(1, 512 / tiles);
    int64_t rpc = (M + want - 1) / want;
    rpc = std::max<int64_t>(min_rows, ((rpc + 63) / 64) * 64);
    return (int)rpc;
}

static int dw_chunk(const papc_sa_plan &p, int l, int a_mode, int dz_mode)
{
    const int64_t M = rows_of(p.d);
    int rpc = 0;
    const bool plain = p.d.input == PAPC_SA_IN_ROWS;
    if (l > 0 || !plain) rpc = papc_mlp_bwd_dw_chunk_hint(M, cin_of(p, l), p.d.cout[l], a_mode, dz_mode, dz_mode == PAPC_DZ_MAX ? p.d.K : 0);
    if (rpc <= 0) rpc = dw_rows_per_chunk(M, p.d.cout[l], cin_of(p, l));
    return rpc;
}

static size_t layout_saved(const papc_sa_plan &p, void *base, SavedPtrs &s)
{
    Carver c{reinterpret_cast<char *>(base), 0};
    const int L = p.d.n_layers;
    const int64_t M = rows_of(p.d), G = (int64_t)p.d.B * p.d.S;
    memset(&s, 0, sizeof(s));
    for (int l = 0; l < L; ++l) {
        const bool stored = !(l == 0 && p.xyz1) && !(l == L - 1 && p.nostore);
        s.y[l] = stored ? c.take<float>((size_t)M * p.d.cout[l] + 64) : nullptr;
        s.cst[l] = c.take<float>(4 * (size_t)p.d.cout[l]);
    }
    if (p.d.pool) {
        s.argmax = c.take<int32_t>((size_t)G * p.d.cout[L - 1]);
        if (p.gmax || p.compact) s.gbuf_f = c.take<float>(2 * (size_t)G * p.d.cout[L - 1]);
    }
    if (p.xyz1) {
        s.xc = c.take<float>((size_t)M * 4);
        s.gram = c.take<double>(16);
        s.wf = c.take<float>(4 * (size_t)p.d.cout[0]);
    }
    if (p.lin0) s.P = c.take<float>((size_t)p.d.B * p.d.N * p.d.cout[0]);
    return c.off;
}

static size_t layout_fwd(const papc_sa_plan &p, void *base, FwdPtrs &f)
{
    Carver c{reinterpret_cast<char *>(base), 0};
    const int L = p.d.n_layers;
    const int64_t M = rows_of(p.d), G = (int64_t)p.d.B * p.d.S;
    memset(&f, 0, sizeof(f));
    int cmax = 0;
    for (int l = 0; l < L; ++l) cmax = std::max(cmax, p.d.cout[l]);
    const int rows = std::max(papc_mlp_gemm_parts(M), p.lin0 ? papc_lingather_parts(M) : 0) + (p.compact ? papc_compact_corr_parts() : 0);
    f.stats = c.take<float>((size_t)rows * 2 * cmax * L);
    if (p.gmax) f.gbuf_i = c.take<int32_t>(2 * (size_t)G * p.d.cout[L - 1]);
    if (p.lin0) f.wfeat = c.take<float>((size_t)p.d.cout[0] * p.d.D);
    if (p.xyz1) f.gpart = c.take<double>((size_t)papc_xyz_parts(M) * 16 + 16);
    return c.off;
}

static size_t layout_bwd(const papc_sa_plan &p, void *base, BwdPtrs &b)
{
    Carver c{reinterpret_cast<char *>(base), 0};
    const int L = p.d.n_layers;
    const int64_t M = rows_of(p.d), G = (int64_t)p.d.B * p.d.S;
    memset(&b, 0, sizeof(b));
    int cmax = p.cin0;
    for (int l = 0; l < L; ++l) cmax = std::max(cmax, p.d.cout[l]);
    const int n_parts = (int)std::min<int64_t>(512, (M + 127) / 128);
    const int gparts = papc_mlp_gemm_parts(M);
    for (int l = 0; l < L; ++l) {
        const int cin = cin_of(p, l), cout = p.d.cout[l];
        b.c12[l] = c.take<float>(2 * (size_t)cout);
        b.wt[l] = c.take<float>((size_t)cin * cout);
        const int dzm = (l == L - 1 && p.d.pool) ? PAPC_DZ_MAX : PAPC_DZ_DENSE;
        const int am = l == 0 ? (p.d.input == PAPC_SA_IN_ROWS ? A_PLAIN_ : A_GROUP_) : ((l == 1 && p.xyz1) ? A_XYZ_ : A_BNRELU_);
        const int rpc = dw_chunk(p, l, am, dzm);
        const int64_t n_chunks = (M + rpc - 1) / rpc;
        b.part[l] = c.take<float>((size_t)n_chunks * ((size_t)cout * cin + cout));
    }
    b.red = c.take<float>((size_t)n_parts * 2 * cmax);
    b.fused_red[0] = c.take<float>((size_t)gparts * 2 * cmax);
    b.fused_red[1] = c.take<float>((size_t)gparts * 2 * cmax);
    if (L > 1 || p.d.input == PAPC_SA_IN_ROWS) {
        b.dz[0] = c.take<float>((size_t)M * cmax + 64);
        if (L > 2) b.dz[1] = c.take<float>((size_t)M * cmax + 64);
    }
    if (p.d.pool && L > 1) {
        const int cL = p.d.cout[L - 1], cLi = p.d.cout[L - 2];
        b.psel = c.take<float>((size_t)G * cL);
        b.wcat = c.take<float>((size_t)cLi * (cL + cLi));
        b.hb = c.take<float>((size_t)cLi);
        b.eq = c.take<float>(2 * (size_t)cL);
        if (p.nostore) b.dwmax_ws = c.take<float>((size_t)papc_mlp_bwd_dw_max_ws_floats(M, cLi, cL) + 4);
    }
    if (p.xyz1) b.bpart = c.take<float>((size_t)std::max(papc_xyz_bwd_parts(M), papc_mlp_gemm_parts(M)) * p.d.cout[0] * 4);
    if (p.lin0) {
        const int c0 = p.d.cout[0];
        const int64_t BN = (int64_t)p.d.B * p.d.N;
        b.dwx_part = c.take<float>((size_t)std::max(papc_lingather_parts(M), papc_lingather_list_parts(BN)) * c0 * 3);
        b.Gs = c.take<float>((size_t)BN * c0);
        const int rpc_g = dw_rows_per_chunk(BN, c0, p.d.D, 64);
        b.part_g = c.take<float>((size_t)((BN + rpc_g - 1) / rpc_g) * ((size_t)c0 * p.d.D + c0));
        b.wft = c.take<float>((size_t)p.d.D * c0);
    }
    b.tmp_gb = c.take<float>(2 * (size_t)cmax);
    return c.off;
}

constexpr int PG_GROUP = 128, PG_MAX_ROWS = 16384;
struct PlanesSaved {
    float *y[PAPC_SA_MAX_LAYERS], *cst[PAPC_SA_MAX_LAYERS];
    int32_t *argmax; float *gbuf_f;
    float *ysel;
    void *PT[PAPC_SA_MAX_LAYERS];
    void *wtp[PAPC_SA_MAX_LAYERS];
};
struct PlanesFwd { void *wp[PAPC_SA_MAX_LAYERS]; void *P; float *stats[PAPC_SA_MAX_LAYERS]; int32_t *gbuf_i; };
struct PlanesBwd { void *dyp, *dypt; float *dz[2], *red[3], *part[PAPC_SA_MAX_LAYERS], *tmp_gb; };

static int pg_split_for(int R1, int R2, int nst)
{
    const int tiles = ((R1 + 127) / 128) * ((R2 + 127) / 128);
    int s = 1;
    const int min_stages = tiles <= 2 ? 2 : 8;
    while (s * 2 * tiles <= 256 && nst % (s * 2) == 0 && nst / (s * 2) >= min_stages) s *= 2;
    return s;
}
static inline int pg_n_in(const papc_sa_plan &p) { return p.d.input == PAPC_SA_IN_ROWS ? p.cin0 : p.d.D; }

static size_t layout_planes_saved(const papc_sa_plan &p, void *base, PlanesSaved &s)
{
    Carver c{reinterpret_cast<char *>(base), 0};
    const int L = p.d.n_layers;
    const int64_t M = rows_of(p.d), T = M / PG_GROUP;
    memset(&s, 0, sizeof(s));
    for (int l = 0; l < L; ++l) {
        s.y[l] = c.take<float>((size_t)M * p.d.cout[l]);
// ... 272 lines not shown
    return PAPC_OK;
}

int papc_sa_mlp_fwd(const papc_sa_plan *plan, const papc_sa_io *io, papc_stream_t st)
{
    PAPC_REQUIRE(plan && io && io->out && io->saved && io->scratch, PAPC_E_INVALID, "papc_sa_mlp_fwd: null pointer");
    const papc_sa_plan &p = *plan;
    const papc_sa_desc &d = p.d;
    const int L = d.n_layers;
    const int64_t M = rows_of(d), G = (int64_t)d.B * d.S;
    const bool plain = d.input == PAPC_SA_IN_ROWS, ev = d.eval_bn != 0;
    PAPC_REQUIRE(plain ? io->x_rows != nullptr : (io->xyz && io->new_xyz), PAPC_E_INVALID, "papc_sa_mlp_fwd: missing input");
    PAPC_REQUIRE(plain || d.identity_rows || io->idx, PAPC_E_INVALID, "papc_sa_mlp_fwd: grouped input without idx (set identity_rows for sample_and_group_all)");
    PAPC_REQUIRE(plain || d.D == 0 || io->feats, PAPC_E_INVALID, "papc_sa_mlp_fwd: D = %d but feats is NULL", d.D);
    PAPC_REQUIRE(!p.compact || io->compact, PAPC_E_INVALID, "papc_sa_mlp_fwd: the plan is compacted but io->compact is NULL");
    if (p.planes) {
        for (int l = 0; l < L; ++l) PAPC_REQUIRE(io->layer[l].w && io->layer[l].gamma && io->layer[l].beta, PAPC_E_INVALID, "papc_sa_mlp_fwd: layer %d lacks w / gamma / beta", l);
        return planes_fwd(p, *io, st);
    }
    SavedPtrs s; FwdPtrs f;
    layout_saved(p, io->saved, s);
    layout_fwd(p, io->scratch, f);
    const int parts = papc_mlp_gemm_parts(M);
    const bool wstats = p.compact && !(d.disable & PAPC_SA_NO_WSTATS);
    const int R_c = (p.compact && !wstats) ? papc_compact_corr_parts() : 0;
    papc_group_src grp;
    if (!plain) fill_grp(grp, d, *io, p.compact);
    if (!plain && wstats) grp.wstat = io->compact->wrow;
    int cmax = 0;
    for (int l = 0; l < L; ++l) cmax = std::max(cmax, d.cout[l]);
    const size_t stats_stride = (size_t)(std::max(parts, p.lin0 ? papc_lingather_parts(M) : 0) + R_c) * 2 * cmax;

    const float *prev_y = nullptr, *prev_sc = nullptr, *prev_sh = nullptr;
    int cin = p.cin0;
    const float *xc = nullptr;
    papc_group_max gm;
    memset(&gm, 0, sizeof(gm));
    for (int l = 0; l < L; ++l) {
        const papc_sa_layer &ly = io->layer[l];
        PAPC_REQUIRE(ly.w && ly.gamma && ly.beta, PAPC_E_INVALID, "papc_sa_mlp_fwd: layer %d lacks w / gamma / beta", l);
        PAPC_REQUIRE(!ev || (ly.running_mean && ly.running_var), PAPC_E_INVALID, "papc_sa_mlp_fwd: eval_bn needs the running statistics");
        const int cout = d.cout[l];
        float *stats = ev ? nullptr : f.stats + (size_t)l * stats_stride;
        int parts_l = parts;
        const papc_group_max *gm_ref = nullptr;
        if (l == L - 1 && p.gmax) {
            gm.gmax = s.gbuf_f; gm.gmin = s.gbuf_f + G * cout; gm.amax = f.gbuf_i; gm.amin = f.gbuf_i + G * cout; gm.K = d.K;
            gm.sign_src = (d.disable & PAPC_SA_NO_GSIGN) ? nullptr : ly.gamma;
            gm_ref = &gm;
        }
        float *y = s.y[l];
        float *cst = s.cst[l];
        if (l == 0 && p.xyz1) {
            const double *gpart1;
            if (io->xc && io->xc_gram) { xc = io->xc; gpart1 = io->xc_gram; }
            else {
                SA_CALL(papc_xyz_group_f32(&grp, d.B, s.xc, f.gpart + 16, st));
                SA_CALL(papc_xyz_gram_fold_f32(f.gpart + 16, papc_xyz_parts(M), f.gpart, st));
                xc = s.xc; gpart1 = f.gpart;
            }
            SA_CALL(papc_xyz_l1_finalize_f32(gpart1, 1, M, ly.w, cin, 0, ly.b, ly.gamma, ly.beta, d.eps, d.momentum, cout, cst, cst + cout, cst + 2 * cout,
                                             cst + 3 * cout, ly.running_mean, ly.running_var, s.wf, s.gram, st));
            prev_y = nullptr; prev_sc = cst + 2 * cout; prev_sh = cst + 3 * cout;
            cin = cout;
            continue;
        }
        if (l == 1 && p.xyz1) {
            SA_CALL(papc_mlp_gemm_f32(A_XYZ_, xc, 4, nullptr, s.wf, nullptr, ly.w, ly.b, M, cin, cout, y, stats, gm_ref, st));
        } else if (l == 0 && plain) {
            SA_CALL(papc_mlp_gemm_f32(A_PLAIN_, io->x_rows, cin, nullptr, nullptr, nullptr, ly.w, ly.b, M, cin, cout, y, stats, gm_ref, st));
        } else if (l == 0 && p.lin0) {
            const int fcol0 = d.xyz_first ? 3 : 0;
            const float *wfeat = io->wfeat;
            if (!wfeat) {
                SA_CALL(papc_copy2d_f32(ly.w + fcol0, cin, f.wfeat, d.D, cout, d.D, 0, st));
                wfeat = f.wfeat;
            }
            const int64_t BN = (int64_t)d.B * d.N;
            SA_CALL(papc_mlp_gemm_f32(A_PLAIN_, io->feats, d.D, nullptr, nullptr, nullptr, wfeat, nullptr, BN, d.D, cout, s.P, nullptr, nullptr, st));
            parts_l = papc_lingather_parts(M);
            SA_CALL(papc_lingather_fwd_f32(s.P, &grp, d.B, ly.w, cin, d.xyz_first ? 0 : d.D, ly.b, cout, y, stats, st));
        } else if (l == 0) {
            SA_CALL(papc_mlp_gemm_f32(A_GROUP_, nullptr, 0, &grp, nullptr, nullptr, ly.w, ly.b, M, cin, cout, y, stats, gm_ref, st));
        } else if (p.compact) {
            SA_CALL(papc_mlp_gemm_rows_w_f32(A_BNRELU_, prev_y, cin, nullptr, prev_sc, prev_sh, ly.w, ly.b, M, cin, cout, y, stats, nullptr, io->compact->rows,
                                             wstats ? io->compact->wrow : nullptr, st));
        } else {
            SA_CALL(papc_mlp_gemm_f32(A_BNRELU_, prev_y, cin, nullptr, prev_sc, prev_sh, ly.w, ly.b, M, cin, cout, y, stats, gm_ref, st));
        }
        if (p.compact && !wstats) {
            SA_CALL(papc_bn_stats_corr_f32(y, cout, io->compact->start, io->compact->coef, io->compact->G, stats + (size_t)parts_l * 2 * cout, st));
            parts_l += R_c;
        }
        if (ev) SA_CALL(papc_bn_eval_consts_f32(ly.running_mean, ly.running_var, ly.gamma, ly.beta, d.eps, cout, cst, cst + cout, cst + 2 * cout, cst + 3 * cout, st));
        else SA_CALL(papc_bn_finalize_f32(stats, parts_l, M, cout, ly.gamma, ly.beta, d.eps, d.momentum, cst, cst + cout, cst + 2 * cout, cst + 3 * cout,
                                          ly.running_mean, ly.running_var, st));
        prev_y = y; prev_sc = cst + 2 * cout; prev_sh = cst + 3 * cout;
        cin = cout;
    }
    if (!d.pool) return papc_bn_relu_f32(prev_y, prev_sc, prev_sh, M, cin, io->out, st);
    if (p.compact) return papc_bn_relu_max_seg_f32(prev_y, cin, io->compact->start, prev_sc, prev_sh, (int)G, io->out, s.argmax, s.gbuf_f, st);
    if (p.gmax) return papc_bn_select_max_f32(s.gbuf_f, s.gbuf_f + G * cin, f.gbuf_i, f.gbuf_i + G * cin, prev_sc, prev_sh, G, cin, io->out, s.argmax, st);
    return papc_bn_relu_max_f32(prev_y, prev_sc, prev_sh, G, d.K, cin, io->out, s.argmax, st);
}

int papc_sa_mlp_bwd(const papc_sa_plan *plan, const papc_sa_io *io, const papc_sa_grads *gr, papc_stream_t st)
{
    PAPC_REQUIRE(plan && io && gr && gr->gout && io->saved && io->scratch, PAPC_E_INVALID, "papc_sa_mlp_bwd: null pointer");
    const papc_sa_plan &p = *plan;
    const papc_sa_desc &d = p.d;
    const int L = d.n_layers;
    const int64_t M = rows_of(d), G = (int64_t)d.B * d.S;
    const bool plain = d.input == PAPC_SA_IN_ROWS, ev = d.eval_bn != 0;
    if (p.planes) return planes_bwd(p, *io, *gr, st);
    SavedPtrs s; BwdPtrs b;
    layout_saved(p, io->saved, s);
    layout_bwd(p, io->scratch, b);
    const float *xc = p.xyz1 ? ((io->xc && io->xc_gram) ? io->xc : s.xc) : nullptr;
    papc_group_src grp;
    if (!plain) fill_grp(grp, d, *io, p.compact);
    const int n_parts = (int)std::min<int64_t>(512, (M + 127) / 128);
    const int gemm_parts = papc_mlp_gemm_parts(M);
    const bool x_needs = plain && gr->grad_x, f_needs = !plain && d.D > 0 && gr->grad_feats && !d.cut_gather_grad;
    const float *ysel = (p.gmax || p.compact) ? s.gbuf_f : nullptr;
    const float *ones = io->consts3, *zeros = nullptr, *big = nullptr;
    int cmaxc = 0;
    for (int l = 0; l < L; ++l) cmaxc = std::max(cmaxc, d.cout[l]);
    if (p.lin0) {
        PAPC_REQUIRE(io->consts3 && io->consts3_ld >= d.cout[0], PAPC_E_INVALID, "papc_sa_mlp_bwd: the gather-add first layer needs consts3 (ones | zeros | 1e30 rows of >= %d floats)", d.cout[0]);
        zeros = io->consts3 + io->consts3_ld; big = io->consts3 + 2 * (int64_t)io->consts3_ld;
    }

    bool need_wt[PAPC_SA_MAX_LAYERS];
    const float *wts[PAPC_SA_MAX_LAYERS];
    for (int l = 0; l < L; ++l) {
        need_wt[l] = l > 0 || x_needs || f_needs;
        wts[l] = nullptr;
    }
    if (p.sparse_max) need_wt[L - 1] = false;
    if (p.lin0) need_wt[0] = false;
    {
        const float *srcs[8]; float *dsts[8]; int rws[8], cls[8];
        int n = 0;
        for (int l = 0; l < L; ++l) {
            if (!need_wt[l]) continue;
            if (gr->wt[l]) { wts[l] = gr->wt[l]; continue; }
            srcs[n] = io->layer[l].w; dsts[n] = b.wt[l]; rws[n] = d.cout[l]; cls[n] = cin_of(p, l);
            wts[l] = b.wt[l];
            if (++n == 8) { SA_CALL(papc_transpose_batch_f32(srcs, dsts, rws, cls, n, st)); n = 0; }
        }
        if (n) SA_CALL(papc_transpose_batch_f32(srcs, dsts, rws, cls, n, st));
    }

    papc_reduce_job jobs[PAPC_SA_MAX_LAYERS];
    int n_jobs = 0;
    bool xyz_fused = false;
    bool dz0_masked = false;
    const float *dz = nullptr;
    const float *fused_red = nullptr;
    int flip = 0;
    for (int l = L - 1; l >= 0; --l) {
        const papc_sa_layer &ly = io->layer[l];
        const int cout = d.cout[l], cin = cin_of(p, l);
        const float *cst = s.cst[l];
        float *c12 = b.c12[l];
        const bool acc_w = gr->acc_w[l] != 0, acc_gb = gr->acc_gb[l] != 0 && !ev;
        float *dgamma = gr->dgamma[l] ? gr->dgamma[l] : b.tmp_gb, *dbeta = gr->dbeta[l] ? gr->dbeta[l] : b.tmp_gb + cmaxc;
        PAPC_REQUIRE(gr->dw[l], PAPC_E_INVALID, "papc_sa_mlp_bwd: dw[%d] is NULL", l);
        papc_bwd_dy dy;
        memset(&dy, 0, sizeof(dy));
        if (p.compact) { dy.wrow = io->compact->wrow; dy.seg_grp = io->compact->seg_grp; dy.rows_dev = io->compact->rows; }
        if (l == L - 1 && !d.pool) { dy.dz_mode = PAPC_DZ_DENSE; dy.dz = gr->gout; dy.K = 1; }
        else if (l == L - 1) { dy.dz_mode = PAPC_DZ_MAX; dy.gout = gr->gout; dy.argmax = s.argmax; dy.K = d.K; }
        else { dy.dz_mode = PAPC_DZ_DENSE; dy.dz = dz; dy.K = 1; }
        if (l == 0 && p.xyz1) {
            PAPC_REQUIRE(!gr->dgamma[l] || (gr->acc_gb[l] != 0) == (gr->acc_w[l] != 0), PAPC_E_UNSUPPORTED,
                         "papc_sa_mlp_bwd: the coordinates-only first layer takes ONE accumulate flag for dw / dgamma / dbeta");
            int nbp = papc_xyz_bwd_parts(M);
            if (xyz_fused) nbp = papc_mlp_gemm_parts(M);
            else SA_CALL(papc_xyz_l1_bwd_f32(dz, xc, s.wf, M, cout, b.bpart, st));
            SA_CALL(papc_xyz_l1_bwd_finalize_f32(b.bpart, nbp, M, cout, s.gram, ly.w, cin, 0, ly.b, cst, cst + cout, cst + 2 * cout, dgamma, dbeta, gr->dw[l],
                                                 acc_w ? 1 : 0, st));
            if (gr->db[l] && !acc_w) SA_CALL(papc_fill_f32(gr->db[l], cout, 0.f, st));
// ... 204 lines not shown
```

papc_amd/mlp.py:

```python
import ctypes

import torch

from . import _lib
from ._lib import BwdDy, BwdRed, GroupMax, GroupSrc, ReduceJob, ScatterDst, check, ptr, stream_ptr

A_PLAIN, A_BNRELU, A_GROUP, A_XYZ = 0, 1, 2, 6
DZ_DENSE, DZ_MAX = 0, 1


class StackSpec:

    def __init__(self, B, N, S, K, D, xyz_first, eps=1e-5, momentum=0.9, cut_gather_grad=False, pool=True, eval_bn=False):
        self.B, self.N, self.S, self.K, self.D = B, N, S, K, D
        self.pool = bool(pool)
        self.eval_bn = bool(eval_bn)
        self.xyz_first = bool(xyz_first)
        self.eps, self.momentum = float(eps), float(momentum)
        self.cut_gather_grad = cut_gather_grad
        self.M = B * S * K
        self.grad_targets = None
        self.wt_table = None
        self.xyz_pre = None
        self.compact = None
# ... 41 lines not shown
    st = stream_ptr()
    table = {}
    ok = lambda w: w.is_cuda and w.is_contiguous() and w.dtype == torch.float32
    jobs = []
    for w in weights:
        if ok(w):
            cout = w.shape[0]
            cin = w.numel() // cout
            t = torch.empty(cin, cout, device=w.device, dtype=torch.float32)
            table[w.data_ptr()] = t
            jobs.append((w.data_ptr(), cin, t, cout, cin, 0))
    for w, xyz_first in feat_blocks:
        cout = w.shape[0]
        cin = w.numel() // cout
        if ok(w) and cin > 3:
            t = torch.empty(cout, cin - 3, device=w.device, dtype=torch.float32)
            table[("f", w.data_ptr())] = (t, bool(xyz_first))
            jobs.append((w.data_ptr() + (12 if xyz_first else 0), cin, t, cout, cin - 3, 1))
    for g0 in range(0, len(jobs), 8):
        grp = jobs[g0:g0 + 8]
        n = len(grp)
        srcs, dsts = (ctypes.c_void_p * n)(), (ctypes.c_void_p * n)()
        lds, rws, cls, cps = (ctypes.c_int * n)(), (ctypes.c_int * n)(), (ctypes.c_int * n)(), (ctypes.c_int * n)()
        for i, (src, ld, t, rows, cols, cp) in enumerate(grp):
            srcs[i], lds[i], dsts[i], rws[i], cls[i], cps[i] = src, ld, t.data_ptr(), rows, cols, cp
        check(lib.papc_transpose_batch_ld_f32(srcs, lds, dsts, rws, cls, cps, n, st), "papc_transpose_batch_ld_f32")
    return table


def xyz_first_layer_ok(M, c1, c2, n_layers):
    return bool(_XYZ1 and n_layers >= 3 and _lib.load().papc_mlp_xyz_ok(M, c1, c2))


def xyz_pregroup(xyz, new_xyz, idx, out=None):
    lib = _lib.load()
    B, N = xyz.shape[0], xyz.shape[1]
    S, K = idx.shape[1], idx.shape[2]
    M = B * S * K
    dev = xyz.device
    if out is None:
        out = (torch.empty(M, 4, device=dev, dtype=torch.float32), torch.empty(1, 16, device=dev, dtype=torch.float64))
    gpart = torch.empty(lib.papc_xyz_parts(M), 16, device=dev, dtype=torch.float64)
    g = GroupSrc()
    g.xyz = xyz.data_ptr()
    g.sb, g.sn, g.sc = xyz.stride(0), xyz.stride(1), xyz.stride(2)
    g.new_xyz, g.feats, g.idx = new_xyz.data_ptr(), 0, idx.data_ptr()
    g.N, g.S, g.K, g.D, g.xyz_first = N, S, K, 0, 1
    check(lib.papc_xyz_group_f32(ctypes.byref(g), B, ptr(out[0]), ptr(gpart), stream_ptr()), "papc_xyz_group_f32")
    check(lib.papc_xyz_gram_fold_f32(ptr(gpart), gpart.shape[0], ptr(out[1]), stream_ptr()), "papc_xyz_gram_fold_f32")
    return out


class SharedMLPMax(torch.autograd.Function):

    @staticmethod
    def forward(ctx, spec, bn_buffers, xyz, new_xyz, feats, idx, x_rows, *params):
        lib = _lib.load()
        st = stream_ptr()
        dev = params[0].device
        L = len(params) // 4
        M = spec.M
        parts = lib.papc_mlp_gemm_parts(M)
        plain = x_rows is not None
        grp = None if plain else _group_src(spec, xyz, new_xyz, feats, idx)
        ys, consts = [], []
        prev_y, prev_sc, prev_sh = None, None, None
        cin = x_rows.shape[1] if plain else spec.D + 3
        cin0 = cin
        ev = spec.eval_bn
        assert not ev or bn_buffers is not None, "eval_bn needs the running statistics"
        lin0 = (_LIN_GATHER and not ev and not plain and idx is not None and feats is not None and L >= 2 and spec.D % 4 == 0 and spec.D >= 16
                and params[0].shape[0] % 4 == 0 and params[0].shape[0] <= 256 and feats.is_contiguous())
        xyz1 = (not ev and not plain and idx is not None and feats is None and spec.D == 0
                and xyz_first_layer_ok(M, params[0].shape[0], params[4].shape[0] if L >= 2 else 0, L))
        xc = wf = gram = None
        cp = spec.compact if (lin0 and spec.pool and spec.compact is not None) else None
        if cp is not None:
            from . import compact as _cpm
            if not _cpm.stack_ok(M, spec.K, [params[4 * l].shape[0] for l in range(L)]):
                cp = None
        R_c = lib.papc_compact_corr_parts() if cp is not None else 0
        if cp is not None:
            grp.cidx, grp.seg_grp, grp.rows_dev = cp.cidx.data_ptr(), cp.seg_grp.data_ptr(), cp.rows.data_ptr()
        for l in range(L):
            w, b, gamma, beta = params[4 * l: 4 * l + 4]
            cout = w.shape[0]
            w2 = w.reshape(cout, cin)
            assert w2.is_contiguous()
            stats = None if ev else torch.empty(parts + R_c, 2, cout, device=dev, dtype=torch.float32)
            parts_l = parts
            gm_ref = None
            if cp is None and l == L - 1 and spec.pool and _FUSE_GMAX and not ev and lib.papc_mlp_gemm_gmax_ok(M, cout, spec.K):
                G_ = M // spec.K
                gbuf_f = torch.empty(2, G_, cout, device=dev, dtype=torch.float32)
                gbuf_i = torch.empty(2, G_, cout, device=dev, dtype=torch.int32)
                gm = GroupMax()
                gm.gmax, gm.gmin = gbuf_f[0].data_ptr(), gbuf_f[1].data_ptr()
                gm.amax, gm.amin = gbuf_i[0].data_ptr(), gbuf_i[1].data_ptr()
                gm.K = spec.K
                gm_ref = ctypes.byref(gm)
            if (gm_ref is not None and _NOSTORE and L >= 2 and l == L - 1 and prev_y is not None and not (l == 1 and xyz1)
                    and lib.papc_mlp_max_nostore_ok(M, cin, cout, spec.K)):
                y = None
            else:
                y = None if (l == 0 and xyz1) else torch.empty(M, cout, device=dev, dtype=torch.float32)
            if l == 0 and xyz1:
                y = stats = None
                nparts = 1
                if spec.xyz_pre is not None:
                    xc, gpart = spec.xyz_pre
                    assert tuple(xc.shape) == (M, 4) and tuple(gpart.shape) == (1, 16)
                else:
                    xc, gpart = xyz_pregroup(xyz, new_xyz, idx)
                cst = torch.empty(4, cout, device=dev, dtype=torch.float32)
                wf = torch.empty(cout, 4, device=dev, dtype=torch.float32)
                gram = torch.empty(16, device=dev, dtype=torch.float64)
                rm, rv = (bn_buffers[l] if bn_buffers is not None else (None, None))
                check(lib.papc_xyz_l1_finalize_f32(ptr(gpart), nparts, M, ptr(w2), cin, 0, ptr(b), ptr(gamma), ptr(beta), spec.eps, spec.momentum,
                                                   cout, cst[0].data_ptr(), cst[1].data_ptr(), cst[2].data_ptr(), cst[3].data_ptr(), ptr(rm), ptr(rv),
                                                   ptr(wf), ptr(gram), st), "papc_xyz_l1_finalize_f32")
                ys.append(None)
                consts.append(cst)
                prev_y, prev_sc, prev_sh = None, cst[2], cst[3]
                cin = cout
                continue
            if l == 1 and xyz1:
                check(lib.papc_mlp_gemm_f32(A_XYZ, ptr(xc), 4, None, ptr(wf), None, ptr(w2), ptr(b), M, cin, cout,
                                            ptr(y), ptr(stats), gm_ref, st), "papc_mlp_gemm_f32")
            elif l == 0 and plain:
                check(lib.papc_mlp_gemm_f32(A_PLAIN, ptr(x_rows), cin, None, None, None, ptr(w2), ptr(b), M, cin, cout,
                                            ptr(y), ptr(stats), gm_ref, st), "papc_mlp_gemm_f32")
            elif l == 0 and lin0:
                fcol0 = 3 if spec.xyz_first else 0
                wf = torch.empty(cout, spec.D, device=dev, dtype=torch.float32)
                check(lib.papc_copy2d_f32(w2.data_ptr() + 4 * fcol0, cin, ptr(wf), spec.D, cout, spec.D, 0, st), "papc_copy2d_f32")
                BN_ = spec.B * spec.N
                P = torch.empty(BN_, cout, device=dev, dtype=torch.float32)
                check(lib.papc_mlp_gemm_f32(A_PLAIN, ptr(feats), spec.D, None, None, None, ptr(wf), None, BN_, spec.D, cout, ptr(P), None,
                                            None, st), "papc_mlp_gemm_f32")
                parts_l = lib.papc_lingather_parts(M)
                stats = torch.empty(parts_l + R_c, 2, cout, device=dev, dtype=torch.float32)
                check(lib.papc_lingather_fwd_f32(ptr(P), ctypes.byref(grp), spec.B, ptr(w2), cin, 0 if spec.xyz_first else spec.D,
                                                 ptr(b), cout, ptr(y), ptr(stats), st), "papc_lingather_fwd_f32")
            elif l == 0:
                check(lib.papc_mlp_gemm_f32(A_GROUP, None, 0, ctypes.byref(grp), None, None, ptr(w2), ptr(b), M, cin, cout,
                                            ptr(y), ptr(stats), gm_ref, st), "papc_mlp_gemm_f32")
            elif cp is not None:
                check(lib.papc_mlp_gemm_rows_f32(A_BNRELU, ptr(prev_y), cin, None, ptr(prev_sc), ptr(prev_sh), ptr(w2), ptr(b), M, cin,
                                                 cout, ptr(y), ptr(stats), None, cp.rows.data_ptr(), st), "papc_mlp_gemm_rows_f32")
            else:
                check(lib.papc_mlp_gemm_f32(A_BNRELU, ptr(prev_y), cin, None, ptr(prev_sc), ptr(prev_sh), ptr(w2), ptr(b), M, cin,
                                            cout, ptr(y), ptr(stats), gm_ref, st), "papc_mlp_gemm_f32")
            if cp is not None:
                check(lib.papc_bn_stats_corr_f32(ptr(y), cout, cp.start.data_ptr(), cp.coef.data_ptr(), cp.G,
                                                 stats.data_ptr() + 4 * parts_l * 2 * cout, st), "papc_bn_stats_corr_f32")
                parts_l += R_c
            cst = torch.empty(4, cout, device=dev, dtype=torch.float32)
            rm, rv = (bn_buffers[l] if bn_buffers is not None else (None, None))
            if ev:
                check(lib.papc_bn_eval_consts_f32(ptr(rm), ptr(rv), ptr(gamma), ptr(beta), spec.eps, cout, cst[0].data_ptr(),
                                                  cst[1].data_ptr(), cst[2].data_ptr(), cst[3].data_ptr(), st), "papc_bn_eval_consts_f32")
            else:
                check(lib.papc_bn_finalize_f32(ptr(stats), parts_l, M, cout, ptr(gamma), ptr(beta), spec.eps, spec.momentum,
                                               cst[0].data_ptr(), cst[1].data_ptr(), cst[2].data_ptr(), cst[3].data_ptr(),
                                               ptr(rm), ptr(rv), st), "papc_bn_finalize_f32")
            ys.append(y)
            consts.append(cst)
            prev_y, prev_sc, prev_sh = y, cst[2], cst[3]
            cin = cout
        G = spec.B * spec.S
        argmax = None
        if not spec.pool:
            out = torch.empty(M, cin, device=dev, dtype=torch.float32)
            check(lib.papc_bn_relu_f32(ptr(prev_y), ptr(prev_sc), ptr(prev_sh), M, cin, ptr(out), st), "papc_bn_relu_f32")
        else:
            out = torch.empty(G, cin, device=dev, dtype=torch.float32)
            argmax = torch.empty(G, cin, device=dev, dtype=torch.int32)
        ysel_c = None
        if not spec.pool:
            pass
        elif cp is not None:
            ysel_c = torch.empty(G, cin, device=dev, dtype=torch.float32)
            check(lib.papc_bn_relu_max_seg_f32(ptr(prev_y), cin, cp.start.data_ptr(), ptr(prev_sc), ptr(prev_sh), G, ptr(out), ptr(argmax),
                                               ptr(ysel_c), st), "papc_bn_relu_max_seg_f32")
        elif gm_ref is not None:
            check(lib.papc_bn_select_max_f32(gbuf_f[0].data_ptr(), gbuf_f[1].data_ptr(), gbuf_i[0].data_ptr(), gbuf_i[1].data_ptr(),
                                             ptr(prev_sc), ptr(prev_sh), G, cin, ptr(out), ptr(argmax), st), "papc_bn_select_max_f32")
        else:
            check(lib.papc_bn_relu_max_f32(ptr(prev_y), ptr(prev_sc), ptr(prev_sh), G, spec.K, cin, ptr(out), ptr(argmax), st),
                  "papc_bn_relu_max_f32")
        ctx.spec = spec
        ctx.L = L
        ctx.wt_table = spec.wt_table
        ctx.feats_needs_grad = feats is not None and feats.requires_grad and not spec.cut_gather_grad
        ctx.x_needs_grad = plain and x_rows.requires_grad
        ctx.cin0 = cin0
        ctx.lin0 = lin0
        ctx.xyz1 = xyz1
        ctx.nostore = spec.pool and L >= 1 and ys[L - 1] is None and not (xyz1 and L == 1)
        ysel = gbuf_f[0] if (spec.pool and gm_ref is not None) else ysel_c
        ctx.compact = cp
        if xyz1:
            ys[0] = xc
            consts = consts + [wf, gram]
        ctx.save_for_backward(xyz, new_xyz, feats, idx, x_rows, argmax, ysel, *params, *ys, *consts)
        return out

    @staticmethod
    def backward(ctx, gout):
        lib = _lib.load()
        st = stream_ptr()
        spec, L = ctx.spec, ctx.L
        saved = ctx.saved_tensors
        xyz, new_xyz, feats, idx, x_rows, argmax, ysel = saved[:7]
        params = saved[7:7 + 4 * L]
        ys = saved[7 + 4 * L: 7 + 5 * L]
        consts = saved[7 + 5 * L: 7 + 6 * L]
        xyz1 = ctx.xyz1
        xc = wf = gram = None
        if xyz1:
            xc, (wf, gram) = ys[0], saved[7 + 6 * L: 7 + 6 * L + 2]
        plain = x_rows is not None
        dev = gout.device
        M = spec.M
        gout = gout.contiguous().float()
        grp = None if plain else _group_src(spec, xyz, new_xyz, feats, idx)
        cp = ctx.compact
        if cp is not None:
            grp.cidx, grp.seg_grp, grp.rows_dev = cp.cidx.data_ptr(), cp.seg_grp.data_ptr(), cp.rows.data_ptr()
        n_parts = min(_RESIDENT_WGS, (M + 127) // 128)
        grads = [None] * (4 * L)
        reduce_jobs = []
        grad_feats = None
        grad_x = None
        dz = None
        fused_red = None
        gemm_parts = lib.papc_mlp_gemm_parts(M)
        need_wt = [l for l in range(L) if l > 0 or (plain and ctx.x_needs_grad) or ((not plain) and ctx.feats_needs_grad)]
        cL, cLi = params[4 * (L - 1)].shape[0], (params[4 * (L - 2)].shape[0] if L > 1 else 0)
        sparse_max = ctx.nostore or (_SPARSE_MAX and spec.pool and L > 1 and ysel is not None and M >= 32768 and cL % 16 == 0 and cLi % 4 == 0
                                     and cL + cLi <= 512)
        max_prep = None
        if sparse_max:
            need_wt.remove(L - 1)
        if ctx.lin0 and 0 in need_wt:
            need_wt.remove(0)
        wts = {}
        if ctx.wt_table is not None:
            for l in list(need_wt):
                t = ctx.wt_table.get(params[4 * l].data_ptr())
                cin_l = ctx.cin0 if l == 0 else params[4 * (l - 1)].shape[0]
                if t is not None and tuple(t.shape) == (cin_l, params[4 * l].shape[0]):
                    wts[l] = t
                    need_wt.remove(l)
        for g0 in range(0, len(need_wt), 8):
            grp_l = need_wt[g0:g0 + 8]
            n = len(grp_l)
            srcs, dsts, rws, cls = (ctypes.c_void_p * n)(), (ctypes.c_void_p * n)(), (ctypes.c_int * n)(), (ctypes.c_int * n)()
            for i, l in enumerate(grp_l):
                w = params[4 * l]
                cout = w.shape[0]
                cin = ctx.cin0 if l == 0 else params[4 * (l - 1)].shape[0]
                assert w.is_contiguous()
# ... 246 lines not shown
```

papc_amd/stack.py:

```python
import ctypes
import os

import torch

from . import _lib
from ._lib import check, ptr, stream_ptr

MAXL = 8
c_p, c_i, c_l, c_f = ctypes.c_void_p, ctypes.c_int32, ctypes.c_int64, ctypes.c_float
NO_LINGATHER, NO_XYZ1, NO_NOSTORE, NO_GMAX, NO_FUSED_RED, NO_COMPACT, NO_PLANES, NO_PLANES_POINTWISE, NO_XYZ_FUSE, NO_WSTATS, NO_PSEL, NO_GSIGN = 1, 2, 4, 8, 16, 32, 64, 128, 256, 512, 1024, 2048


class SaDesc(ctypes.Structure):
    _fields_ = [("B", c_i), ("N", c_i), ("S", c_i), ("K", c_i), ("D", c_i), ("n_layers", c_i), ("cin", c_i), ("cout", c_i * MAXL),
                ("input", c_i), ("identity_rows", c_i), ("xyz_first", c_i), ("pool", c_i), ("eval_bn", c_i), ("cut_gather_grad", c_i),
                ("eps", c_f), ("momentum", c_f), ("disable", ctypes.c_uint32), ("inference", c_i), ("want_input_grad", c_i)]


class SaLayer(ctypes.Structure):
    _fields_ = [("w", c_p), ("b", c_p), ("gamma", c_p), ("beta", c_p), ("running_mean", c_p), ("running_var", c_p)]


class CompactSrc(ctypes.Structure):
    _fields_ = [("start", c_p), ("rows", c_p), ("cidx", c_p), ("seg_grp", c_p), ("wrow", c_p), ("coef", c_p), ("G", c_i)]


class SaIo(ctypes.Structure):
    _fields_ = [("xyz", c_p), ("sb", c_l), ("sn", c_l), ("sc", c_l), ("new_xyz", c_p), ("feats", c_p), ("idx", c_p), ("x_rows", c_p),
                ("xc", c_p), ("xc_gram", c_p), ("compact", ctypes.POINTER(CompactSrc)), ("consts3", c_p), ("consts3_ld", c_i),
                ("layer", SaLayer * MAXL), ("out", c_p), ("saved", c_p), ("scratch", c_p), ("plists", c_p), ("wfeat", c_p)]


class SaPlan(ctypes.Structure):
    _fields_ = [("d", SaDesc), ("cin0", c_i), ("lin0", c_i), ("xyz1", c_i), ("gmax", c_i), ("nostore", c_i), ("compact", c_i), ("sparse_max", c_i),
                ("planes", c_i), ("saved_bytes", c_l), ("fwd_scratch_bytes", c_l), ("bwd_scratch_bytes", c_l), ("off_y", c_l * MAXL), ("off_cst", c_l * MAXL),
                ("off_argmax", c_l)]


class SaGrads(ctypes.Structure):
    _fields_ = [("gout", c_p), ("dw", c_p * MAXL), ("db", c_p * MAXL), ("dgamma", c_p * MAXL), ("dbeta", c_p * MAXL), ("acc_w", c_i * MAXL),
                ("acc_gb", c_i * MAXL), ("wt", c_p * MAXL), ("grad_feats", c_p), ("grad_x", c_p), ("defer", c_p)]


_CONSTS3 = {}
LAST_PLANS = {}


def _consts3(dev):
    t = _CONSTS3.get(str(dev))
    if t is None:
        mk = lambda: torch.tensor([1.0, 0.0, 1e30], device=dev, dtype=torch.float32).view(3, 1).expand(3, 1024).contiguous()
        if _lib._capturing():
            return mk()
        t = _CONSTS3[str(dev)] = mk()
    return t


def _disable_bits():
    from . import mlp
    bits = 0
    if not mlp._LIN_GATHER: bits |= NO_LINGATHER
    if not mlp._XYZ1: bits |= NO_XYZ1
    if not mlp._NOSTORE: bits |= NO_NOSTORE
    if not mlp._FUSE_GMAX: bits |= NO_GMAX
    if not mlp._FUSE_RED: bits |= NO_FUSED_RED
    from . import smallm
    if not smallm.ENABLED: bits |= NO_PLANES
    if not smallm.POINTWISE: bits |= NO_PLANES_POINTWISE
    if not mlp._XYZ_FUSE: bits |= NO_XYZ_FUSE
    if os.environ.get("PAPC_GSIGN", "1") == "0": bits |= NO_GSIGN
    if os.environ.get("PAPC_PSEL", "1") == "0": bits |= NO_PSEL
    if os.environ.get("PAPC_WSTATS", "1") == "0": bits |= NO_WSTATS
    return bits


def _fill_io(io, spec, xyz, new_xyz, feats, idx, x_rows, params, bn_buffers, keep):
    L = len(params) // 4
    if x_rows is None:
        io.xyz = xyz.data_ptr()
        io.sb, io.sn, io.sc = xyz.stride(0), xyz.stride(1), xyz.stride(2)
        io.new_xyz, io.feats, io.idx = new_xyz.data_ptr(), ptr(feats), ptr(idx)
    else:
        io.x_rows = x_rows.data_ptr()
    if spec.xyz_pre is not None:
        io.xc, io.xc_gram = spec.xyz_pre[0].data_ptr(), spec.xyz_pre[1].data_ptr()
    cp = spec.compact
    if cp is not None:
        src = CompactSrc(cp.start.data_ptr(), cp.rows.data_ptr(), cp.cidx.data_ptr(), cp.seg_grp.data_ptr(), cp.wrow.data_ptr(), cp.coef.data_ptr(), cp.G)
        keep.append(src)
        io.compact = ctypes.pointer(src)
    pl = getattr(spec, "plists", None)
    if pl is not None:
        src = _lib.PointLists(pl.prange.data_ptr(), pl.prow.data_ptr(), pl.pmeta.data_ptr(), int(pl.compact),
                              pl.pmom.data_ptr() if getattr(pl, "pmom", None) is not None else None)
        keep.append(src)
        keep.append(pl)
        io.plists = ctypes.addressof(src)
    wtab = getattr(spec, "wt_table", None)
    if wtab is not None and feats is not None and L >= 1:
        ent = wtab.get(("f", params[0].data_ptr()))
        cin0 = params[0].numel() // params[0].shape[0]
        if ent is not None and ent[1] == bool(spec.xyz_first) and tuple(ent[0].shape) == (params[0].shape[0], cin0 - 3) and cin0 - 3 == spec.D:
            io.wfeat = ent[0].data_ptr()
            keep.append(ent[0])
    c3 = _consts3(params[0].device)
    keep.append(c3)
    io.consts3, io.consts3_ld = c3.data_ptr(), c3.shape[1]
    for l in range(L):
        w, b, gamma, beta = params[4 * l: 4 * l + 4]
        ly = io.layer[l]
        assert w.is_contiguous()
        ly.w, ly.b, ly.gamma, ly.beta = w.data_ptr(), ptr(b), gamma.data_ptr(), beta.data_ptr()
        if bn_buffers is not None:
            ly.running_mean, ly.running_var = ptr(bn_buffers[l][0]), ptr(bn_buffers[l][1])


class SharedMLPStack(torch.autograd.Function):

    @staticmethod
    def forward(ctx, spec, bn_buffers, xyz, new_xyz, feats, idx, x_rows, *params):
        lib = _lib.load()
        dev = params[0].device
        L = len(params) // 4
        assert 1 <= L <= MAXL
        plain = x_rows is not None
        d = SaDesc()
        d.B, d.N, d.S, d.K, d.D, d.n_layers = spec.B, spec.N, spec.S, spec.K, spec.D, L
        d.cin = x_rows.shape[1] if plain else spec.D + 3
        for l in range(L):
            d.cout[l] = params[4 * l].shape[0]
        d.input = 1 if plain else 0
        d.identity_rows = int((not plain) and idx is None)
        d.xyz_first, d.pool, d.eval_bn, d.cut_gather_grad = int(spec.xyz_first), int(spec.pool), int(spec.eval_bn), int(bool(spec.cut_gather_grad))
        d.eps, d.momentum = spec.eps, spec.momentum
        d.disable = _disable_bits()
        if feats is not None and not feats.is_contiguous():
            d.disable |= NO_LINGATHER | NO_PLANES
        if plain and not x_rows.is_contiguous():
            d.disable |= NO_PLANES
        d.inference = int(not any(ctx.needs_input_grad))
        d.want_input_grad = int((plain and x_rows.requires_grad) or ((not plain) and feats is not None and feats.requires_grad and not spec.cut_gather_grad))
        keep = []
        io = SaIo()
        _fill_io(io, spec, xyz, new_xyz, feats, idx, x_rows, params, bn_buffers, keep)
        plan = SaPlan()
        check(lib.papc_sa_mlp_plan(ctypes.byref(d), ctypes.byref(io), ctypes.byref(plan)), "papc_sa_mlp_plan")
        M = spec.M
        G = spec.B * spec.S
        cL = params[4 * (L - 1)].shape[0]
        out = torch.empty(G if spec.pool else M, cL, device=dev, dtype=torch.float32)
        saved = torch.empty(plan.saved_bytes, device=dev, dtype=torch.uint8)
        scratch = torch.empty(plan.fwd_scratch_bytes, device=dev, dtype=torch.uint8)
        io.out, io.saved, io.scratch = out.data_ptr(), saved.data_ptr(), scratch.data_ptr()
        check(lib.papc_sa_mlp_fwd(ctypes.byref(plan), ctypes.byref(io), stream_ptr()), "papc_sa_mlp_fwd")
        ctx.spec, ctx.L, ctx.plan, ctx.saved = spec, L, plan, saved
# ... 86 lines not shown
```

Measured before the change: 21650.

## Emit per-8-row segment max records from last-layer GEMM epilogue for compacted max-pool

Measured after the change: 21900, median of 6. 1.1% higher.

```diff
diff --git a/include/papc_hip.h b/include/papc_hip.h
--- a/include/papc_hip.h
+++ b/include/papc_hip.h
@@ -214,6 +214,7 @@
 #define PAPC_SA_NO_PSEL 1024u
 #define PAPC_SA_NO_GSIGN 2048u
 #define PAPC_SA_NO_WSTATS 512u
+#define PAPC_SA_NO_SEGREC 4096u
 typedef struct papc_sa_desc {
     int32_t B, N, S, K, D;
     int32_t n_layers;
@@ -402,6 +403,12 @@
 int papc_bn_stats_corr_f32(const float *y, int C, const int32_t *start, const float *coef, int G, float *stats_rows, papc_stream_t stream);
 int papc_bn_relu_max_seg_f32(const float *y, int C, const int32_t *start, const float *scale, const float *shift, int G, float *out,
                              int32_t *argmax, float *ysel, papc_stream_t stream);
+int papc_mlp_segrec_ok(int64_t M, int Cin, int Cout);
+int papc_mlp_gemm_rows_seg_f32(const float *x, int64_t ldx, const float *bn_scale, const float *bn_shift, const float *w, const float *bias,
+                               int64_t M, int Cin, int Cout, float *y, float *stats_partial, const int32_t *rows_dev, const float *wrow,
+                               const float *sign_src, float *seg_key, int32_t *seg_off, papc_stream_t stream);
+int papc_bn_relu_max_segrec_f32(const float *y, int C, const int32_t *start, const float *scale, const float *shift, const float *sign_src,
+                                const float *seg_key, const int32_t *seg_off, int G, float *out, int32_t *argmax, float *ysel, papc_stream_t stream);
 int papc_lingather_fwd_f32(const float *P, const papc_group_src *grp, int B, const float *w, int ldw, int xcol0, const float *bias, int C,
                            float *y, float *stats_partial, papc_stream_t stream);
 int papc_lingather_bwd_f32(const papc_bwd_dy *dy, const papc_group_src *grp, int B, int C, float *G, float *dwx_partial, papc_stream_t stream);
diff --git a/papc_amd/_lib.py b/papc_amd/_lib.py
--- a/papc_amd/_lib.py
+++ b/papc_amd/_lib.py
@@ -87,6 +87,9 @@
     "papc_mlp_compact_ok": (c_i, [c_l, c_i, c_i, c_p]),
     "papc_bn_stats_corr_f32": (c_i, [c_p, c_i, c_p, c_p, c_i, c_p, c_p]),
     "papc_bn_relu_max_seg_f32": (c_i, [c_p, c_i, c_p, c_p, c_p, c_i, c_p, c_p, c_p, c_p]),
+    "papc_mlp_segrec_ok": (c_i, [c_l, c_i, c_i]),
+    "papc_mlp_gemm_rows_seg_f32": (c_i, [c_p, c_l, c_p, c_p, c_p, c_p, c_l, c_i, c_i, c_p, c_p, c_p, c_p, c_p, c_p, c_p, c_p]),
+    "papc_bn_relu_max_segrec_f32": (c_i, [c_p, c_i, c_p, c_p, c_p, c_p, c_p, c_p, c_i, c_p, c_p, c_p, c_p]),
     "papc_bn_select_max_f32": (c_i, [c_p, c_p, c_p, c_p, c_p, c_p, c_l, c_i, c_p, c_p, c_p]),
     "papc_bn_finalize_f32": (c_i, [c_p, c_i, c_l, c_i, c_p, c_p, c_f, c_f, c_p, c_p, c_p, c_p, c_p, c_p, c_p]),
     "papc_bn_relu_max_f32": (c_i, [c_p, c_p, c_p, c_l, c_i, c_i, c_p, c_p, c_p]),
diff --git a/papc_amd/csrc/compact.hip b/papc_amd/csrc/compact.hip
--- a/papc_amd/csrc/compact.hip
+++ b/papc_amd/csrc/compact.hip
@@ -166,6 +166,74 @@
     *reinterpret_cast<float4 *>(ysel + q) = make_float4(ys[0], ys[1], ys[2], ys[3]);
 }
 
+__global__ __launch_bounds__(256) void seg_max_rec_kernel(const float *__restrict__ y, int C, const int32_t *__restrict__ start,
+                                                          const float *__restrict__ scale, const float *__restrict__ shift,
+                                                          const float *__restrict__ sgn, const float *__restrict__ seg_key,
+                                                          const int32_t *__restrict__ seg_off, int G, float *__restrict__ out,
+                                                          int32_t *__restrict__ argmax, float *__restrict__ ysel)
+{
+    const int CQ = C >> 2;
+    const int64_t e = (int64_t)blockIdx.x * 256 + threadIdx.x;
+    if (e >= (int64_t)G * CQ) return;
+    const int g = (int)(e / CQ), c = (int)(e - (int64_t)g * CQ) * 4;
+    const int r0 = start[g], r1 = start[g + 1];
+    const float4 sc = *reinterpret_cast<const float4 *>(scale + c), sh = *reinterpret_cast<const float4 *>(shift + c);
+    const float4 gs = *reinterpret_cast<const float4 *>(sgn + c);
+    const float s4[4] = {sc.x, sc.y, sc.z, sc.w}, h4[4] = {sh.x, sh.y, sh.z, sh.w}, g4[4] = {gs.x, gs.y, gs.z, gs.w};
+    int flip[4];
+    bool same = true;
+#pragma unroll
+    for (int i = 0; i < 4; ++i) {
+        flip[i] = s4[i] >= 0.f ? 0 : (int)0x80000000u;
+        same = same && ((g4[i] >= 0.f) == (s4[i] >= 0.f));
+    }
+    float mx[4] = {-INFINITY, -INFINITY, -INFINITY, -INFINITY};
+    int ix[4] = {r0, r0, r0, r0};
+    if (same) {
+        auto take = [&](int s, const float4 &k, const int4 &o) {
+            const float kk[4] = {k.x, k.y, k.z, k.w};
+            const int oo[4] = {o.x, o.y, o.z, o.w};
+            const int sh8 = (s & 3) * 8;
+#pragma unroll
+            for (int i = 0; i < 4; ++i)
+                if (kk[i] > mx[i]) { mx[i] = kk[i]; ix[i] = 8 * s + ((oo[i] >> sh8) & 7); }
+        };
+        const int s1 = r1 >> 3;
+        int s = r0 >> 3;
+        for (; s + 4 <= s1; s += 4) {
+            float4 k[4];
+            int4 o[4];
+#pragma unroll
+            for (int u = 0; u < 4; ++u) {
+                k[u] = *reinterpret_cast<const float4 *>(seg_key + (int64_t)(s + u) * C + c);
+                o[u] = *reinterpret_cast<const int4 *>(seg_off + (int64_t)((s + u) >> 2) * C + c);
+            }
+#pragma unroll
+            for (int u = 0; u < 4; ++u) take(s + u, k[u], o[u]);
+        }
+        for (; s < s1; ++s)
+            take(s, *reinterpret_cast<const float4 *>(seg_key + (int64_t)s * C + c), *reinterpret_cast<const int4 *>(seg_off + (int64_t)(s >> 2) * C + c));
+    } else {
+        for (int r = r0; r < r1; ++r) {
+#pragma unroll
+            for (int i = 0; i < 4; ++i) {
+                const float k = __int_as_float(__float_as_int(y[(int64_t)r * C + c + i]) ^ flip[i]);
+                if (k > mx[i]) { mx[i] = k; ix[i] = r; }
+            }
+        }
+    }
+    float o[4], ys[4];
+#pragma unroll
+    for (int i = 0; i < 4; ++i) {
+        ys[i] = __int_as_float(__float_as_int(mx[i]) ^ flip[i]);
+        o[i] = relu_np(fmaf(s4[i], ys[i], h4[i]));
+    }
+    const int64_t q = (int64_t)g * C + c;
+    *reinterpret_cast<float4 *>(out + q) = make_float4(o[0], o[1], o[2], o[3]);
+    *reinterpret_cast<int4 *>(argmax + q) = make_int4(ix[0], ix[1], ix[2], ix[3]);
+    *reinterpret_cast<float4 *>(ysel + q) = make_float4(ys[0], ys[1], ys[2], ys[3]);
+}
+
 }
 
 using namespace papc;
@@ -212,4 +280,19 @@
     return check_launch("papc_bn_relu_max_seg_f32");
 }
 
-}
+int papc_bn_relu_max_segrec_f32(const float *y, int C, const int32_t *start, const float *scale, const float *shift, const float *sign_src,
+                                const float *seg_key, const int32_t *seg_off, int G, float *out, int32_t *argmax, float *ysel, papc_stream_t stream)
+{
+    PAPC_REQUIRE(y && start && scale && shift && sign_src && seg_key && seg_off && out && argmax && ysel, PAPC_E_INVALID,
+                 "papc_bn_relu_max_segrec_f32: null pointer");
+    PAPC_REQUIRE(G >= 1 && C >= 4 && C % 4 == 0, PAPC_E_UNSUPPORTED, "papc_bn_relu_max_segrec_f32: C=%d must be a multiple of 4", C);
+    PAPC_REQUIRE(aligned16(scale) && aligned16(shift) && aligned16(sign_src) && aligned16(seg_key) && aligned16(seg_off) && aligned16(out) &&
+                 aligned16(argmax) && aligned16(ysel), PAPC_E_INVALID, "papc_bn_relu_max_segrec_f32: 16-byte alignment");
+    hipStream_t st = as_stream(stream);
+    ProfScope prof(PAPC_K_BN_RELU_MAX, st);
+    hipLaunchKernelGGL(seg_max_rec_kernel, dim3((unsigned)cdiv((int64_t)G * (C / 4), 256)), dim3(256), 0, st, y, C, start, scale, shift, sign_src,
+                       seg_key, seg_off, G, out, argmax, ysel);
+    return check_launch("papc_bn_relu_max_segrec_f32");
+}
+
+}
diff --git a/papc_amd/csrc/mlp_gemm.h b/papc_amd/csrc/mlp_gemm.h
--- a/papc_amd/csrc/mlp_gemm.h
+++ b/papc_amd/csrc/mlp_gemm.h
@@ -37,6 +37,7 @@
     GmaxDst gm;
     const int32_t *rows_dev;
     const float *wstat;
+    float *segk; int32_t *sego;
     unsigned long long *dbg;
     int tl;
 };
diff --git a/papc_amd/csrc/mlp_gemm.hip b/papc_amd/csrc/mlp_gemm.hip
--- a/papc_amd/csrc/mlp_gemm.hip
+++ b/papc_amd/csrc/mlp_gemm.hip
@@ -966,6 +966,35 @@
     }
 }
 
+int papc_mlp_segrec_ok(int64_t M, int Cin, int Cout)
+{
+    if (!knob(KNOB_STREAM) || knob(KNOB_GEMM_F32) || !knob(KNOB_STREAM_ASM)) return 0;
+    return (Cin == 128 && Cout == 256 && M % 128 == 0 && M / 32 >= knob(KNOB_STREAM_MINTILES)) ? 1 : 0;
+}
+
+int papc_mlp_gemm_rows_seg_f32(const float *x, int64_t ldx, const float *bn_scale, const float *bn_shift, const float *w, const float *bias,
+                               int64_t M, int Cin, int Cout, float *y, float *stats_partial, const int32_t *rows_dev, const float *wrow,
+                               const float *sign_src, float *seg_key, int32_t *seg_off, papc_stream_t stream)
+{
+    PAPC_REQUIRE(x && w && y && stats_partial && rows_dev && sign_src && seg_key && seg_off, PAPC_E_INVALID, "papc_mlp_gemm_rows_seg_f32: null pointer");
+    PAPC_REQUIRE(papc_mlp_segrec_ok(M, Cin, Cout), PAPC_E_UNSUPPORTED, "papc_mlp_gemm_rows_seg_f32: not built for M=%lld Cin=%d Cout=%d",
+                 (long long)M, Cin, Cout);
+    GemmArgs p;
+    memset(&p, 0, sizeof(p));
+    int rc = fill_asrc(p.a, A_BNRELU, x, ldx, nullptr, bn_scale, bn_shift, Cin, "papc_mlp_gemm_rows_seg_f32");
+    if (rc) return rc;
+    p.w = w; p.ldw = Cin; p.bias = bias; p.M = M; p.Kin = Cin; p.Nout = Cout; p.y = y; p.ldy = Cout; p.stats = stats_partial;
+    p.rows_dev = rows_dev; p.wstat = wrow;
+    p.gm.sgn = sign_src; p.segk = seg_key; p.sego = seg_off;
+    p.parts = gemm_parts(M);
+    const bool vec = p.a.vec && aligned16(w) && aligned16(y);
+    hipStream_t st = as_stream(stream);
+    ProfScope prof(PAPC_K_MLP_GEMM, st);
+    const int rc2 = stream_gemm_try(p, A_BNRELU, EPI_STORE, vec, st);
+    if (rc2 == 0) { set_error("papc_mlp_gemm_rows_seg_f32: the row-streaming kernel declined M=%lld Cin=%d Cout=%d (alignment?)", (long long)M, Cin, Cout); return PAPC_E_UNSUPPORTED; }
+    return rc2 < 0 ? rc2 : PAPC_OK;
+}
+
 int papc_mlp_gemm_rows_f32(int a_mode, const float *x, int64_t ldx, const papc_group_src *grp,
                            const float *bn_scale, const float *bn_shift, const float *w, const float *bias,
                            int64_t M, int Cin, int Cout, float *y, float *stats_partial, const papc_group_max *gmax,
diff --git a/papc_amd/csrc/mlp_stream.hip b/papc_amd/csrc/mlp_stream.hip
--- a/papc_amd/csrc/mlp_stream.hip
+++ b/papc_amd/csrc/mlp_stream.hip
@@ -61,10 +61,11 @@
 }
 
 template <int AMODE, int EPI, int KB16, int CK, int WN, bool ASM, bool CP = false, int KV = KB16 * 16, bool NR = false, int CBW = WN * 32, bool PS = false, int NWT = 8,
-          bool GS = false>
+          bool GS = false, bool SR = false>
 __global__ __launch_bounds__(NWT * 64, NWT / 4) void stream_kernel(GemmArgs p, StreamGeo geo)
 {
     static_assert(!GS || EPI == EPI_STORE_GMAX || EPI == EPI_GMAX, "GS: group-max epilogues only");
+    static_assert(!SR || (EPI == EPI_STORE && AMODE == A_BNRELU && !NR && CBW == WN * 32 && KV == KB16 * 16), "SR: the storing BN+ReLU forward, whole blocks");
     static_assert(NWT == 8 || NWT == 12, "two or three waves per SIMD");
     static_assert(!PS || (CP && AMODE == A_DY_MAX), "PS: the compacted max-layer dX only (the one flavour where the result is bit-identical)");
     static_assert(!CP || ((AMODE == A_DY_DENSE || AMODE == A_DY_MAX) && EPI == EPI_STORE_RED && ASM && PAPC_STREAM_PK), "CP: dX flavours of the asm ring only");
@@ -476,6 +477,7 @@
         if (EPI == EPI_STORE_RED) { rsc[wn] = p.rd.scale[col]; rsh[wn] = p.rd.shift[col]; rmu[wn] = p.rd.mean[col]; ris[wn] = p.rd.invstd[col]; }
         gmx[wn] = -INFINITY; gmn[wn] = INFINITY; gix[wn] = 0; gin[wn] = 0;
         if constexpr (GS) gin[wn] = (p.gm.sgn[col] < 0.f) ? (int)0x80000000u : 0;
+        if constexpr (SR) gin[wn] = (p.gm.sgn[col] >= 0.f) ? 0 : (int)0x80000000u;
     }
 
     auto epilogue = [&](int row0, int sub) {
@@ -526,6 +528,10 @@
                 }
                 }
             } else {
+                float sk[4];
+                int so[4];
+#pragma unroll
+                for (int q = 0; q < 4; ++q) { sk[q] = -INFINITY; so[q] = 0; }
 #pragma unroll
                 for (int r = 0; r < 16; ++r) {
                     const int ro = (r & 3) + 8 * (r >> 2);
@@ -533,6 +539,10 @@
                     if (EPI != EPI_GMAX && cok) yp[(int64_t)ro * ldy] = v;
                     s1[wn] += v;
                     s2[wn] = fmaf(v, v, s2[wn]);
+                    if constexpr (SR) {
+                        const float key = __int_as_float(__float_as_int(v) ^ gin[wn]);
+                        if (key > sk[r >> 2]) { sk[r >> 2] = key; so[r >> 2] = (r & 3) + 4 * hi; }
+                    }
                     if (GM) {
                         const int off = sub * 32 + ro + 4 * hi;
                         if constexpr (GS) {
@@ -543,6 +553,18 @@
                             if (v < gmn[wn]) { gmn[wn] = v; gin[wn] = off; }
                         }
                     }
+                }
+                if constexpr (SR) {
+#pragma unroll
+                    for (int q = 0; q < 4; ++q) {
+                        const float ok = __shfl_xor(sk[q], 32);
+                        const int oo = __shfl_xor(so[q], 32);
+                        if (ok > sk[q] || (ok == sk[q] && oo < so[q])) { sk[q] = ok; so[q] = oo; }
+                    }
+                    const int64_t sg = (int64_t)(row0 >> 3) + 2 * hi;
+                    p.segk[sg * p.Nout + col] = hi ? sk[2] : sk[0];
+                    p.segk[(sg + 1) * p.Nout + col] = hi ? sk[3] : sk[1];
+                    if (hi == 0) p.sego[(int64_t)(row0 >> 5) * p.Nout + col] = so[0] | (so[1] << 8) | (so[2] << 16) | (so[3] << 24);
                 }
             }
 #pragma unroll
@@ -740,6 +762,16 @@
     if (gx > p.parts) gx = p.parts;
     dim3 grid((unsigned)gx, (unsigned)ncb);
     if constexpr (!CP && EPI == EPI_STORE_RED) { if (p.rd.masked) return 0; }
+    if (p.segk) {
+        if constexpr (AMODE == A_BNRELU && EPI == EPI_STORE && !KR && !NR && CBW == WN * 32) {
+            if (!knob(KNOB_STREAM_ASM)) return 0;
+            hipLaunchKernelGGL((stream_kernel<AMODE, EPI, KB16, CK, WN, true, false, KV, NR, CBW, false, 8, false, true>), grid, dim3(512), 0, st, p, geo);
+            const int rc = check_launch("mlp stream gemm (segment records)");
+            return rc ? rc : 1;
+        } else {
+            return 0;
+        }
+    }
     if constexpr (CP) {
         if (!knob(KNOB_STREAM_ASM)) return 0;
         if constexpr (PS) {
diff --git a/papc_amd/csrc/sa_mlp.hip b/papc_amd/csrc/sa_mlp.hip
--- a/papc_amd/csrc/sa_mlp.hip
+++ b/papc_amd/csrc/sa_mlp.hip
@@ -46,6 +46,7 @@
 struct FwdPtrs {
     float *stats;
     int32_t *gbuf_i;
+    float *segk; int32_t *sego;
     float *P, *wfeat;
     double *gpart;
 };
@@ -118,6 +119,12 @@
     return c.off;
 }
 
+static bool seg_rec(const papc_sa_plan &p)
+{
+    const int L = p.d.n_layers;
+    return p.compact && L >= 2 && !(p.d.disable & PAPC_SA_NO_SEGREC) && papc_mlp_segrec_ok(rows_of(p.d), p.d.cout[L - 2], p.d.cout[L - 1]);
+}
+
 static size_t layout_fwd(const papc_sa_plan &p, void *base, FwdPtrs &f)
 {
     Carver c{reinterpret_cast<char *>(base), 0};
@@ -129,6 +136,10 @@
     const int rows = std::max(papc_mlp_gemm_parts(M), p.lin0 ? papc_lingather_parts(M) : 0) + (p.compact ? papc_compact_corr_parts() : 0);
     f.stats = c.take<float>((size_t)rows * 2 * cmax * L);
     if (p.gmax) f.gbuf_i = c.take<int32_t>(2 * (size_t)G * p.d.cout[L - 1]);
+    if (seg_rec(p)) {
+        f.segk = c.take<float>((size_t)(M / 8) * p.d.cout[L - 1]);
+        f.sego = c.take<int32_t>((size_t)(M / 32) * p.d.cout[L - 1]);
+    }
     if (p.lin0) f.wfeat = c.take<float>((size_t)p.d.cout[0] * p.d.D);
     if (p.xyz1) f.gpart = c.take<double>((size_t)papc_xyz_parts(M) * 16 + 16);
     return c.off;
@@ -567,6 +578,9 @@
             SA_CALL(papc_lingather_fwd_f32(s.P, &grp, d.B, ly.w, cin, d.xyz_first ? 0 : d.D, ly.b, cout, y, stats, st));
         } else if (l == 0) {
             SA_CALL(papc_mlp_gemm_f32(A_GROUP_, nullptr, 0, &grp, nullptr, nullptr, ly.w, ly.b, M, cin, cout, y, stats, gm_ref, st));
+        } else if (p.compact && l == L - 1 && f.segk) {
+            SA_CALL(papc_mlp_gemm_rows_seg_f32(prev_y, cin, prev_sc, prev_sh, ly.w, ly.b, M, cin, cout, y, stats, io->compact->rows,
+                                               wstats ? io->compact->wrow : nullptr, ly.gamma, f.segk, f.sego, st));
         } else if (p.compact) {
             SA_CALL(papc_mlp_gemm_rows_w_f32(A_BNRELU_, prev_y, cin, nullptr, prev_sc, prev_sh, ly.w, ly.b, M, cin, cout, y, stats, nullptr, io->compact->rows,
                                              wstats ? io->compact->wrow : nullptr, st));
@@ -584,6 +598,9 @@
         cin = cout;
     }
     if (!d.pool) return papc_bn_relu_f32(prev_y, prev_sc, prev_sh, M, cin, io->out, st);
+    if (p.compact && f.segk)
+        return papc_bn_relu_max_segrec_f32(prev_y, cin, io->compact->start, prev_sc, prev_sh, io->layer[L - 1].gamma, f.segk, f.sego, (int)G, io->out,
+                                           s.argmax, s.gbuf_f, st);
     if (p.compact) return papc_bn_relu_max_seg_f32(prev_y, cin, io->compact->start, prev_sc, prev_sh, (int)G, io->out, s.argmax, s.gbuf_f, st);
     if (p.gmax) return papc_bn_select_max_f32(s.gbuf_f, s.gbuf_f + G * cin, f.gbuf_i, f.gbuf_i + G * cin, prev_sc, prev_sh, G, cin, io->out, s.argmax, st);
     return papc_bn_relu_max_f32(prev_y, prev_sc, prev_sh, G, d.K, cin, io->out, s.argmax, st);
diff --git a/papc_amd/mlp.py b/papc_amd/mlp.py
--- a/papc_amd/mlp.py
+++ b/papc_amd/mlp.py
@@ -147,6 +147,7 @@
         R_c = lib.papc_compact_corr_parts() if cp is not None else 0
         if cp is not None:
             grp.cidx, grp.seg_grp, grp.rows_dev = cp.cidx.data_ptr(), cp.seg_grp.data_ptr(), cp.rows.data_ptr()
+        seg_rec = None
         for l in range(L):
             w, b, gamma, beta = params[4 * l: 4 * l + 4]
             cout = w.shape[0]
@@ -210,6 +211,12 @@
             elif l == 0:
                 check(lib.papc_mlp_gemm_f32(A_GROUP, None, 0, ctypes.byref(grp), None, None, ptr(w2), ptr(b), M, cin, cout,
                                             ptr(y), ptr(stats), gm_ref, st), "papc_mlp_gemm_f32")
+            elif cp is not None and l == L - 1 and os.environ.get("PAPC_SEGREC", "1") == "1" and lib.papc_mlp_segrec_ok(M, cin, cout):
+                segk = torch.empty(M // 8, cout, device=dev, dtype=torch.float32)
+                sego = torch.empty(M // 32, cout, device=dev, dtype=torch.int32)
+                check(lib.papc_mlp_gemm_rows_seg_f32(ptr(prev_y), cin, ptr(prev_sc), ptr(prev_sh), ptr(w2), ptr(b), M, cin, cout, ptr(y), ptr(stats),
+                                                     cp.rows.data_ptr(), None, ptr(gamma), ptr(segk), ptr(sego), st), "papc_mlp_gemm_rows_seg_f32")
+                seg_rec = (gamma, segk, sego)
             elif cp is not None:
                 check(lib.papc_mlp_gemm_rows_f32(A_BNRELU, ptr(prev_y), cin, None, ptr(prev_sc), ptr(prev_sh), ptr(w2), ptr(b), M, cin,
                                                  cout, ptr(y), ptr(stats), None, cp.rows.data_ptr(), st), "papc_mlp_gemm_rows_f32")
@@ -244,6 +251,10 @@
         ysel_c = None
         if not spec.pool:
             pass
+        elif cp is not None and seg_rec is not None:
+            ysel_c = torch.empty(G, cin, device=dev, dtype=torch.float32)
+            check(lib.papc_bn_relu_max_segrec_f32(ptr(prev_y), cin, cp.start.data_ptr(), ptr(prev_sc), ptr(prev_sh), ptr(seg_rec[0]), ptr(seg_rec[1]),
+                                                  ptr(seg_rec[2]), G, ptr(out), ptr(argmax), ptr(ysel_c), st), "papc_bn_relu_max_segrec_f32")
         elif cp is not None:
             ysel_c = torch.empty(G, cin, device=dev, dtype=torch.float32)
             check(lib.papc_bn_relu_max_seg_f32(ptr(prev_y), cin, cp.start.data_ptr(), ptr(prev_sc), ptr(prev_sh), G, ptr(out), ptr(argmax),
diff --git a/papc_amd/stack.py b/papc_amd/stack.py
--- a/papc_amd/stack.py
+++ b/papc_amd/stack.py
@@ -9,6 +9,7 @@
 MAXL = 8
 c_p, c_i, c_l, c_f = ctypes.c_void_p, ctypes.c_int32, ctypes.c_int64, ctypes.c_float
 NO_LINGATHER, NO_XYZ1, NO_NOSTORE, NO_GMAX, NO_FUSED_RED, NO_COMPACT, NO_PLANES, NO_PLANES_POINTWISE, NO_XYZ_FUSE, NO_WSTATS, NO_PSEL, NO_GSIGN = 1, 2, 4, 8, 16, 32, 64, 128, 256, 512, 1024, 2048
+NO_SEGREC = 4096
 
 
 class SaDesc(ctypes.Structure):
@@ -71,6 +72,7 @@
     if os.environ.get("PAPC_GSIGN", "1") == "0": bits |= NO_GSIGN
     if os.environ.get("PAPC_PSEL", "1") == "0": bits |= NO_PSEL
     if os.environ.get("PAPC_WSTATS", "1") == "0": bits |= NO_WSTATS
+    if os.environ.get("PAPC_SEGREC", "1") == "0": bits |= NO_SEGREC
     return bits
 
 
```
